# lyclyc52/Instance_NeRF

Hardware: AMD Instinct MI355X
Metric: Msamples/sec (train+infer) 3D-FRONT 800x800 at 1/2/4/8 MI355X; PSNR parity (higher is better)
Workload: dtype f32; 1 GPU; render 800x800 synthetic 3D-FRONT-like room, hash-grid NeRF L=16 F=2 T=6119864 sigma+rgb (BASELINE configs[1]), one view per step per GPU; parallelism=views sharded over 1 GPU(s), no data-path collective

## Files before the change

### include/inr.h

```cpp
#ifndef INR_H
#define INR_H

#include <stdint.h>

#ifdef __cplusplus
extern "C" {
#endif

#define INR_ABI_VERSION 13
#define INR_MAX_LEVELS 16

enum {
  INR_OK = 0,
  INR_EINVAL = -1,
  INR_ELAUNCH = -2,
  INR_ENODEV = -3
};

typedef void* inr_stream_t;

enum {
  INR_NUMERICS_TABLE_F16 = 1,
  INR_NUMERICS_MLP_F16 = 2
};

typedef struct inr_grid_desc {
  int32_t num_levels;
  int32_t level_dim;
  uint32_t offsets[INR_MAX_LEVELS + 1];
  float scales[INR_MAX_LEVELS];
  uint32_t resolutions[INR_MAX_LEVELS];
  uint32_t hashed[INR_MAX_LEVELS];
} inr_grid_desc;

int inr_abi_version(void);
const char* inr_last_error(void);
int inr_device_info(int32_t device, int64_t* props);
int inr_set_overlap_placement(int32_t on);
int inr_set_march_mode(int32_t mode);

int inr_get_rays(const float* poses, int64_t B, float fx, float fy, float cx, float cy, int32_t W,
                 const int64_t* inds , int64_t n, float* rays_o, float* rays_d, inr_stream_t s);

int inr_sample_training_batch(const float* pose , float fx, float fy, float cx, float cy, int32_t H, int32_t W,
                              const float* image , int32_t channels, const int32_t* mask ,
                              int32_t num_instances, int64_t seed, int64_t step, int64_t n, int64_t* inds ,
                              float* rays_o, float* rays_d, float* rgb , int64_t* labels ,
                              inr_stream_t s);

int inr_near_far_from_aabb(const float* rays_o, const float* rays_d, const float* aabb ,
                           int64_t N, float min_near, float* nears, float* fars, inr_stream_t s);
int inr_near_far_from_aabb_skip(const float* rays_o, const float* rays_d, const float* aabb , int64_t N,
                                float min_near, const int64_t* labels, int64_t ignore_index, float* nears, float* fars,
                                inr_stream_t s);

int inr_morton3D(const int32_t* coords , int64_t N, int32_t* indices, inr_stream_t s);
int inr_morton3D_invert(const int32_t* indices, int64_t N, int32_t* coords , inr_stream_t s);
int inr_packbits(const float* grid, int64_t n_bytes, float thresh, uint8_t* bitfield, inr_stream_t s);

int inr_mark_untrained_grid(const float* poses, int32_t B, float fx, float fy, float cx, float cy, int32_t H,
                            int32_t cascade, float bound, float* grid , inr_stream_t s);
int inr_occ_cell_positions(const int32_t* morton_idx, const float* noise, int64_t n, int32_t H, float cascade_bound,
                           float* xyz , inr_stream_t s);
int inr_occ_update(float* grid , const float* sigma , const int32_t* morton_idx ,
                   int64_t n_cells, int64_t m, float decay, float density_scale, float* tmp, double* mean_sum,
                   inr_stream_t s);
int inr_packbits_mean(const float* grid, int64_t n_cells , const double* mean_sum, float density_thresh,
                      uint8_t* bitfield, float* mean_out , const int32_t* counters ,
                      int32_t n_counters, int32_t counter_stride , double* stats_out ,
                      inr_stream_t s);
int64_t inr_occ_sample_workspace_bytes(int64_t n_cells);
int inr_occ_sample_cells(const float* grid , int64_t n_cells, const float* u ,
                         int64_t n, int32_t* morton_idx , void* workspace, inr_stream_t s);

int inr_march_write_fills_unowned_rows(int64_t N, int32_t sample_cap, int32_t max_steps);
int64_t inr_march_workspace_bytes(int64_t N, int32_t sample_cap);
int inr_march_rays_train_count(const float* rays_o, const float* rays_d, const uint8_t* bitfield,
                               float bound, float dt_gamma, int32_t max_steps, int64_t N,
                               int32_t cascade, int32_t H, const float* nears, const float* fars,
                               const float* noises , int32_t* rays ,
                               int32_t* counter , void* workspace, int32_t sample_cap, inr_stream_t s);
int inr_march_rays_train_write(const float* rays_o, const float* rays_d, const uint8_t* bitfield,
                               float bound, float dt_gamma, int32_t max_steps, int64_t N,
                               int32_t cascade, int32_t H, int64_t M, const float* nears,
                               const float* fars, const float* noises ,
                               const int32_t* rays , float* xyzs ,
                               float* dirs , float* deltas , const void* workspace,
                               int32_t sample_cap, inr_stream_t s);

int inr_march_rays_patch_write(const float* rays_o, const float* rays_d, const uint8_t* bitfield,
                               float bound, float dt_gamma, int32_t max_steps, int64_t N,
                               int32_t cascade, int32_t H, int64_t M, const float* nears,
                               const float* fars, const float* noises ,
                               const int32_t* rays ,
                               float* xyzs, float* dirs , float* deltas,
                               const void* workspace, int32_t sample_cap, int32_t* ray_ids ,
                               int32_t normalise , inr_stream_t s);
int inr_composite_rays_patch_forward(const float* sigmas, const float* rgbs, const float* deltas,
                                     const int32_t* rays, int64_t N, int64_t M, float T_thresh,
                                     const float* extra , int32_t K,
                                     float* weights_sum, float* depth, float* image,
                                     float* extra_out , float* weights ,
                                     uint64_t* skippable ,
                                     inr_stream_t s);
int inr_project_masks_patch(const float* xyzs, const float* weights, const int32_t* rays, int64_t N, int64_t M,
                            const uint32_t* mask_words, int32_t W, int32_t L, int32_t H, const float* bbox ,
                            int32_t k_total, int32_t k_base, int32_t k_count, float* out, inr_stream_t s);

int inr_march_rays(int64_t n_alive, int32_t n_step, const int32_t* rays_alive, const float* rays_t,
                   const float* rays_o, const float* rays_d, float bound, float dt_gamma,
                   int32_t max_steps, int32_t cascade, int32_t H, const uint8_t* bitfield,
                   const float* nears, const float* fars, float* xyzs, float* dirs, float* deltas,
                   inr_stream_t s);
int inr_composite_rays(int64_t n_alive, int32_t n_step, int32_t* rays_alive, float* rays_t,
                       const float* sigmas, const float* rgbs, const float* deltas,
                       float* weights_sum, float* depth, float* image, float T_thresh,
                       const float* extra , float* extra_acc ,
                       int32_t K, inr_stream_t s);
int inr_compact_alive(const int32_t* rays_alive, int64_t n_alive, int32_t* out, int32_t* n_out,
                      inr_stream_t s);

int inr_composite_rays_train_forward(const float* sigmas, const float* rgbs, const float* deltas,
                                     const int32_t* rays, int64_t N, int64_t M, float T_thresh,
                                     const float* extra , int32_t K,
                                     float* weights_sum, float* depth, float* image,
                                     float* extra_out , float* weights ,
                                     int32_t* sample_ray , inr_stream_t s);
int inr_composite_rays_extra_forward(const float* weights , const float* extra , const int32_t* rays,
                                     int64_t N, int64_t M, int32_t K, float* extra_out ,
                                     const int64_t* labels , int32_t n_classes, int64_t ignore_index,
                                     float* grad_pix, void* workspace, float* loss_out, inr_stream_t s);
int inr_composite_rays_train_backward(const float* grad_weights_sum, const float* grad_image,
                                      const float* grad_extra_out , const float* sigmas,
                                      const float* rgbs, const float* extra, const float* deltas,
                                      const int32_t* rays, const float* weights_sum,
                                      const float* image, const float* weights ,
                                      int64_t N, int64_t M, float T_thresh, int32_t K,
                                      float* grad_sigmas, float* grad_rgbs ,
                                      float* grad_extra , const int32_t* total_dev ,
                                      inr_stream_t s);

int inr_grid_encode_forward(const float* x , const float* embeddings ,
                            const inr_grid_desc* desc , int64_t M, float bound,
                            float* out , inr_stream_t s);
int inr_grid_encode_backward(const float* x, const float* grad_out ,
                             const inr_grid_desc* desc , int64_t M, float bound,
                             float* grad_embeddings , inr_stream_t s);

int inr_grid_encode_backward_ordered(const float* x, const float* grad_out, const int32_t* order,
                                     const inr_grid_desc* desc , int64_t M, float bound,
                                     float* grad_embeddings , inr_stream_t s);
int inr_grid_encode_backward_input(const float* x, const float* grad_out , const float* embeddings,
                                   const inr_grid_desc* desc , int64_t M, float bound, float* grad_x,
                                   inr_stream_t s);
int inr_grid_encode_backward_levels(const float* x, const float* grad_out, const int32_t* order,
                                    const inr_grid_desc* desc, int64_t M, float bound, float* grad_embeddings,
                                    int32_t level_lo, int32_t level_hi, inr_stream_t s);

#define INR_GRID_FX_STATE_FLOATS 4192
int inr_grid_encode_backward_levels_fx(const float* x, const float* grad_out, const int32_t* order,
                                       const inr_grid_desc* desc, int64_t M, float bound, float* grad_embeddings,
                                       int32_t level_lo, int32_t level_hi, float* fx_state ,
                                       inr_stream_t s);
int inr_grid_grad_finish_fx(float* grad_embeddings, const inr_grid_desc* desc , int32_t level_lo,
                            int32_t level_hi, float* fx_state, inr_stream_t s);
int inr_grid_fx_update(float* fx_state, int32_t num_levels, float headroom, int32_t sum_bits , inr_stream_t s);
int inr_grid_encode_backward_levels_fx64(const float* x, const float* grad_out, const int32_t* order,
                                         const inr_grid_desc* desc, int64_t M, float bound, float* grad_embeddings,
                                         int64_t* acc64 , int32_t level_lo, int32_t level_hi, float* fx_state,
                                         inr_stream_t s);
int inr_grid_grad_finish_fx64(int64_t* acc64, float* grad_embeddings, const inr_grid_desc* desc , int32_t level_lo,
                              int32_t level_hi, float* fx_state, inr_stream_t s);

int inr_sh_encode_forward(const float* d , int64_t M, int32_t degree, float* out, inr_stream_t s);
int inr_sh_encode_backward(const float* grad_out, const float* d, int64_t M, int32_t degree,
                           float* grad_d, inr_stream_t s);
int inr_sh_table_q(const float* d , int64_t N, float* out , inr_stream_t s);

int64_t inr_nerf_packed_floats(void);
int inr_nerf_pack_weights(const float* sigma_w0, const float* sigma_w1, const float* color_w0,
                          const float* color_w1, const float* color_w2, float* packed , int32_t numerics);
int64_t inr_instance_packed_floats(int32_t K);
int inr_instance_pack_weights(const float* w0, const float* w1, const float* w2, int32_t K,
                              float* packed , int32_t numerics);
int inr_nerf_forward(const float* x, const float* d, int64_t M, const int32_t* n_samples_dev,
                     float bound, const void* embeddings, const inr_grid_desc* desc ,
                     const float* packed , float density_scale, float* sigma, float* rgb,
// ... 167 lines not shown
```

### instance_nerf_amd/_lib.py

```python
import ctypes
import os
from ctypes import POINTER, Structure, c_char_p, c_float, c_int32, c_int64, c_uint32, c_void_p

import torch

_HERE = os.path.dirname(os.path.abspath(__file__))
LIB_PATH = os.environ.get("INR_LIB_PATH") or os.path.join(_HERE, "csrc", "libinr_hip.so")
MAX_LEVELS = 16
GRID_FX_STATE_FLOATS = 4192
NUMERICS_TABLE_F16, NUMERICS_MLP_F16 = 1, 2


class GridDesc(Structure):
    _fields_ = [("num_levels", c_int32), ("level_dim", c_int32),
                ("offsets", c_uint32 * (MAX_LEVELS + 1)), ("scales", c_float * MAX_LEVELS),
                ("resolutions", c_uint32 * MAX_LEVELS), ("hashed", c_uint32 * MAX_LEVELS)]


P = c_void_p
_SIGS = {
    "inr_abi_version": (c_int32, []),
    "inr_last_error": (c_char_p, []),
    "inr_set_overlap_placement": (c_int32, [c_int32]),
    "inr_set_march_mode": (c_int32, [c_int32]),
    "inr_device_info": (c_int32, [c_int32, POINTER(c_int64)]),
    "inr_get_rays": (c_int32, [P, c_int64, c_float, c_float, c_float, c_float, c_int32, P, c_int64, P, P, P]),
    "inr_sample_training_batch": (c_int32, [P, c_float, c_float, c_float, c_float, c_int32, c_int32, P, c_int32, P, c_int32,
                                            c_int64, c_int64, c_int64, P, P, P, P, P, P]),
    "inr_near_far_from_aabb": (c_int32, [P, P, P, c_int64, c_float, P, P, P]),
    "inr_near_far_from_aabb_skip": (c_int32, [P, P, P, c_int64, c_float, P, c_int64, P, P, P]),
    "inr_morton3D": (c_int32, [P, c_int64, P, P]),
    "inr_morton3D_invert": (c_int32, [P, c_int64, P, P]),
    "inr_packbits": (c_int32, [P, c_int64, c_float, P, P]),
    "inr_mark_untrained_grid": (c_int32, [P, c_int32, c_float, c_float, c_float, c_float, c_int32, c_int32, c_float, P, P]),
    "inr_occ_cell_positions": (c_int32, [P, P, c_int64, c_int32, c_float, P, P]),
    "inr_occ_update": (c_int32, [P, P, P, c_int64, c_int64, c_float, c_float, P, P, P]),
    "inr_packbits_mean": (c_int32, [P, c_int64, P, c_float, P, P, P, c_int32, c_int32, P, P]),
    "inr_occ_sample_workspace_bytes": (c_int64, [c_int64]),
    "inr_occ_sample_cells": (c_int32, [P, c_int64, P, c_int64, P, P, P]),
    "inr_march_write_fills_unowned_rows": (c_int32, [c_int64, c_int32, c_int32]),
    "inr_march_workspace_bytes": (c_int64, [c_int64, c_int32]),
    "inr_march_rays_train_count": (c_int32, [P, P, P, c_float, c_float, c_int32, c_int64, c_int32, c_int32,
                                             P, P, P, P, P, P, c_int32, P]),
    "inr_march_rays_train_write": (c_int32, [P, P, P, c_float, c_float, c_int32, c_int64, c_int32, c_int32,
                                             c_int64, P, P, P, P, P, P, P, P, c_int32, P]),
    "inr_march_rays_patch_write": (c_int32, [P, P, P, c_float, c_float, c_int32, c_int64, c_int32, c_int32,
                                             c_int64, P, P, P, P, P, P, P, P, c_int32, P, c_int32, P]),
    "inr_nerf_bwd_packed_floats": (c_int64, []),
    "inr_nerf_pack_weights_device": (c_int32, [P, P, P, P, P, P, P, P]),
    "inr_nerf_forward_train": (c_int32, [P, P, c_int64, c_float, P, POINTER(GridDesc), P, P, P, P, P, P, P, P, P, P]),
    "inr_nerf_backward": (c_int32, [P, P, P, P, P, P, P, c_int64, c_float, P, P, P, P, P, P, P, P]),
    "inr_instance_bwd_packed_floats": (c_int64, []),
    "inr_instance_pack_weights_device": (c_int32, [P, P, P, c_int32, P, P, P]),
    "inr_instance_forward_train": (c_int32, [P, c_int64, c_float, P, POINTER(GridDesc), P, c_int32, P, P, P, P, P]),
    "inr_instance_backward": (c_int32, [P, c_int32, P, P, c_int64, P, P, P, P, P]),
    "inr_nerf_forward_enc": (c_int32, [P, P, c_int64, c_float, P, POINTER(GridDesc), P, P, P, P, P]),
    "inr_nerf_head_backward": (c_int32, [P, P, P, P, c_int64, c_float, P, P, P, P, P, P, P, P, P, P, c_int64, P]),
    "inr_instance_forward_enc": (c_int32, [P, c_int64, P, c_float, P, POINTER(GridDesc), P, c_int32, P, P, P]),
    "inr_instance_head_workspace_bytes": (c_int64, []),
    "inr_instance_head_backward": (c_int32, [P, P, P, P, c_int32, c_int64, c_int64, P, P, P, P, P, P, P, P, P, P, P, c_int64, P]),
    "inr_adam_step_multi": (c_int32, [c_int32, P, P, P, P, P, P, c_float, c_float, c_float, c_int32, c_float, P]),
    "inr_adam_ema_step_multi": (c_int32, [c_int32, P, P, P, P, P, P, c_float, c_float, c_float, c_int32, c_float, P,
                                          c_float, P]),
    "inr_adam_set_hyper": (c_int32, [P, c_int32, c_float, c_float, c_float, c_int32, P, P]),
    "inr_adam_step_multi_dev": (c_int32, [c_int32, P, P, P, P, P, P, c_float, c_float, c_float, P]),
    "inr_copy_multi": (c_int32, [c_int32, P, P, P, P]),
    "inr_adam_set_hyper_ema": (c_int32, [P, c_int32, c_float, c_float, c_float, c_int32, c_float, P, P]),
    "inr_adam_ema_step_multi_dev": (c_int32, [c_int32, P, P, P, P, P, P, c_float, c_float, c_float, P, P]),
    "inr_cross_entropy": (c_int32, [P, P, c_int64, c_int32, c_int64, P, P, P, P]),
    "inr_finish_rays": (c_int32, [P, P, P, P, P, P, c_float, c_float, c_float, c_int64, P, P, P]),
    "inr_finish_rays_mse": (c_int32, [P, P, P, P, P, c_float, c_float, c_float, P, P, c_int64, P, P, P, P, P]),
    "inr_sh_table_q": (c_int32, [P, c_int64, P, P]),
    "inr_nerf_forward_table": (c_int32, [P, P, P, c_int64, c_float, P, POINTER(GridDesc), P, c_float, P, P, c_int32, P]),
    "inr_nerf_forward_table_sliced_workspace_bytes": (c_int64, [c_int64]),
    "inr_nerf_forward_table_sliced": (c_int32, [P, P, P, c_int64, c_float, P, POINTER(GridDesc), P, c_float, P, P, P, P]),
    "inr_composite_rays_patch_forward": (c_int32, [P, P, P, P, c_int64, c_int64, c_float, P, c_int32, P, P, P, P, P, P, P]),
    "inr_project_masks_patch": (c_int32, [P, P, P, c_int64, c_int64, P, c_int32, c_int32, c_int32, P, c_int32, c_int32, c_int32,
                                          P, P]),
    "inr_march_rays": (c_int32, [c_int64, c_int32, P, P, P, P, c_float, c_float, c_int32, c_int32, c_int32,
                                 P, P, P, P, P, P, P]),
    "inr_composite_rays": (c_int32, [c_int64, c_int32, P, P, P, P, P, P, P, P, c_float, P, P, c_int32, P]),
    "inr_compact_alive": (c_int32, [P, c_int64, P, P, P]),
    "inr_composite_rays_extra_forward": (c_int32, [P, P, P, c_int64, c_int64, c_int32, P, P, c_int32, c_int64, P, P, P, P]),
    "inr_composite_rays_train_forward": (c_int32, [P, P, P, P, c_int64, c_int64, c_float, P, c_int32, P, P, P, P, P, P, P]),
    "inr_composite_rays_train_backward": (c_int32, [P, P, P, P, P, P, P, P, P, P, P, c_int64, c_int64, c_float, c_int32,
                                                    P, P, P, P, P]),
    "inr_grid_encode_forward": (c_int32, [P, P, POINTER(GridDesc), c_int64, c_float, P, P]),
    "inr_grid_encode_backward": (c_int32, [P, P, POINTER(GridDesc), c_int64, c_float, P, P]),
    "inr_grid_encode_backward_ordered": (c_int32, [P, P, P, POINTER(GridDesc), c_int64, c_float, P, P]),
    "inr_grid_encode_backward_input": (c_int32, [P, P, P, POINTER(GridDesc), c_int64, c_float, P, P]),
    "inr_grid_encode_backward_levels": (c_int32, [P, P, P, POINTER(GridDesc), c_int64, c_float, P, c_int32, c_int32, P]),
    "inr_grid_encode_backward_levels_fx": (c_int32, [P, P, P, POINTER(GridDesc), c_int64, c_float, P, c_int32, c_int32, P, P]),
    "inr_grid_grad_finish_fx": (c_int32, [P, POINTER(GridDesc), c_int32, c_int32, P, P]),
    "inr_grid_fx_update": (c_int32, [P, c_int32, c_float, c_int32, P]),
    "inr_grid_encode_backward_levels_fx64": (c_int32, [P, P, P, POINTER(GridDesc), c_int64, c_float, P, P, c_int32, c_int32, P, P]),
    "inr_grid_grad_finish_fx64": (c_int32, [P, P, POINTER(GridDesc), c_int32, c_int32, P, P]),
    "inr_sh_encode_forward": (c_int32, [P, c_int64, c_int32, P, P]),
    "inr_sh_encode_backward": (c_int32, [P, P, c_int64, c_int32, P, P]),
    "inr_nerf_packed_floats": (c_int64, []),
    "inr_nerf_pack_weights": (c_int32, [P, P, P, P, P, P, c_int32]),
    "inr_instance_packed_floats": (c_int64, [c_int32]),
    "inr_instance_pack_weights": (c_int32, [P, P, P, c_int32, P, c_int32]),
    "inr_nerf_forward": (c_int32, [P, P, c_int64, P, c_float, P, POINTER(GridDesc), P, c_float, P, P, P, c_int32, P]),
    "inr_nerf_forward_dirs": (c_int32, [P, c_int64, c_float, P, POINTER(GridDesc), P, P, c_int32, P, P]),
    "inr_nerf_forward_lattice": (c_int32, [P, P, P, c_int32, c_int32, c_int32, c_float, P, POINTER(GridDesc), P, P, c_int32,
                                           c_float, P, P]),
    "inr_instance_forward": (c_int32, [P, c_int64, P, c_float, P, POINTER(GridDesc), P, c_int32, P, P]),
    "inr_instance_lattice": (c_int32, [P, P, P, c_int32, c_int32, c_int32, c_float, P, POINTER(GridDesc), P, c_float,
                                       c_float, P, POINTER(GridDesc), P, c_int32, P, P, P, P]),
    "inr_instance_volume_stats": (c_int32, [P, P, c_int32, c_int32, c_int32, c_int32, P, c_int64, P, P, P, P]),
    "inr_mesh_workspace_bytes": (c_int64, [c_int32, c_int32, c_int32, c_int32]),
    "inr_mesh_count": (c_int32, [P, c_int32, c_float, c_float, P, c_int32, c_int32, c_int32, c_int32, c_int32, P, c_int64, P, P]),
    "inr_mesh_emit": (c_int32, [P, c_int32, c_float, c_float, P, c_int32, P, P, P, P, c_int32, c_int32, c_int32, c_float,
                                c_float, c_float, c_int32, P, c_int64, c_int32, c_int32, P, P, P, P, P]),
    "inr_components_workspace_bytes": (c_int64, [c_int32, c_int32, c_int32]),
    "inr_components_label": (c_int32, [P, c_int32, c_int32, c_int32, c_int32, P, c_int64, P, P]),
    "inr_components_filter": (c_int32, [P, P, P, c_int32, c_int32, c_int32, c_int32, c_int32, c_int32, c_int32, P, c_int64,
                                        P, P, P, P, P, P]),
    "inr_pack_mask_bits": (c_int32, [P, P, c_int64, c_int32, c_float, c_int64, P, P]),
    "inr_match_count": (c_int32, [P, P, c_int64, c_int64, c_int32, c_int32, P, P, P, P, P]),
    "inr_match_assign": (c_int32, [P, P, P, P, P, c_int64, c_int64, c_int32, c_int32, P, P, P, P]),
    "inr_roi_align_3d_set_mode": (c_int32, [c_int32]),
    "inr_roi_align_3d_forward": (c_int32, [P, P, P, c_int32, c_int32, c_int32, c_int32, c_int32, c_int64, c_int32,
                                           c_int32, c_int32, c_float, P, P]),
    "inr_roi_align_3d_backward": (c_int32, [P, P, P, c_int32, c_int32, c_int32, c_int32, c_int32, c_int64, c_int32,
                                            c_int32, c_int32, c_float, P, P]),
    "inr_roi_align_3d_backward_workspace_bytes": (c_int64, [c_int32, c_int32, c_int32, c_int32, c_int32, c_int64, c_int32,
                                                            c_int32, c_int32]),
    "inr_roi_align_3d_backward_prefers_workspace": (c_int32, [c_int32, c_int32, c_int32, c_int32, c_int32, c_int64, c_int32,
                                                              c_int32, c_int32, c_int64]),
    "inr_roi_align_3d_backward_ws": (c_int32, [P, P, P, c_int32, c_int32, c_int32, c_int32, c_int32, c_int64, c_int32,
                                               c_int32, c_int32, c_float, P, P, c_int64, P]),
    "inr_nerf_render": (c_int32, [P, P, P, P, c_int64, c_int64, c_float, P, POINTER(GridDesc), P, c_float, c_float,
                                  P, P, P, P, P, c_int32, c_int32, P]),
    "inr_instance_render": (c_int32, [P, P, P, c_int64, c_int64, c_float, P, POINTER(GridDesc), P, c_int32, P, c_int32, P,
                                      c_int32, P]),
    "inr_linear_wgrad_workspace_bytes": (c_int64, []),
    "inr_linear_wgrad": (c_int32, [P, P, c_int64, c_int32, c_int32, P, P, P]),
    "inr_adam_step": (c_int32, [P, P, P, P, c_int64, c_float, c_float, c_float, c_float, c_int32, c_float, P]),
}
EXPORTS = tuple(_SIGS)

ABI_VERSION = 13
INSTANCE_STATS_WORKSPACE_BYTES = 512 * 64 * 8 * 4
_lib = None


def load():
    global _lib
    if _lib is not None:
        return _lib
    if not os.path.exists(LIB_PATH):
        raise RuntimeError(
            f"{LIB_PATH} is missing: build it with `python -m instance_nerf_amd.build` "
            "(or __graft_entry__.build()).  There is no CPU fallback.")
    lib = ctypes.CDLL(LIB_PATH)
    version = getattr(lib, "inr_abi_version", None)
    if version is not None:
        version.restype, version.argtypes = c_int32, []
# ... 61 lines not shown
```

### instance_nerf_amd/csrc/raymarch.hip

```cpp
#include "common.h"

namespace inr {

static thread_local char g_err[512] = "";
int g_field_lds_min = 0;
int g_march_lds_pad = 0;
void set_error(const char* fmt, ...) {
  va_list ap;
  va_start(ap, fmt);
  vsnprintf(g_err, sizeof(g_err), fmt, ap);
  va_end(ap);
}

constexpr int kRayBlock = 256;
constexpr float kSqrt3x2 = 3.4641016151377544f;

__global__ void __launch_bounds__(kRayBlock) k_near_far(const float* __restrict__ rays_o,
                                                        const float* __restrict__ rays_d,
                                                        const float* __restrict__ aabb, int64_t N,
                                                        float min_near, float* __restrict__ nears,
                                                        float* __restrict__ fars,
                                                        const int64_t* __restrict__ labels, int64_t ignore) {
  const int64_t n = (int64_t)blockIdx.x * blockDim.x + threadIdx.x;
  if (n >= N) return;
  float near = -INFINITY, far = INFINITY;
  bool miss = labels != nullptr && labels[n] == ignore;
#pragma unroll
  for (int a = 0; a < 3; ++a) {
    const float o = rays_o[n * 3 + a];
    const float rd = 1.0f / rays_d[n * 3 + a];
    const float t0 = (aabb[a] - o) * rd;
    const float t1 = (aabb[a + 3] - o) * rd;
    const float lo = t0 > t1 ? t1 : t0;
    const float hi = t0 > t1 ? t0 : t1;
    if (a > 0) miss = miss || (near > hi) || (lo > far);
    near = lo > near ? lo : near;
    far = hi < far ? hi : far;
  }
  if (near < min_near) near = min_near;
  nears[n] = miss ? 3.402823466e+38f : near;
  fars[n] = miss ? 3.402823466e+38f : far;
}

__global__ void __launch_bounds__(kRayBlock) k_get_rays(const float* __restrict__ poses, int64_t B, float fx, float fy,
                                                        float cx, float cy, int W, const int64_t* __restrict__ inds,
                                                        int64_t n, float* __restrict__ rays_o,
                                                        float* __restrict__ rays_d) {
  const int64_t idx = (int64_t)blockIdx.x * blockDim.x + threadIdx.x;
  if (idx >= B * n) return;
  const int64_t b = idx / n, k = idx - b * n;
  const int64_t pix = inds ? inds[k] : k;
  const float i = (float)(pix % W) + 0.5f, j = (float)(pix / W) + 0.5f;
  const float xs = (i - cx) / fx, ys = (j - cy) / fy;
  const float nrm = sqrtf(xs * xs + ys * ys + 1.0f * 1.0f);
  const float dx = xs / nrm, dy = ys / nrm, dz = 1.0f / nrm;
  const float* P = poses + b * 16;
#pragma unroll
  for (int r = 0; r < 3; ++r) {
    rays_d[idx * 3 + r] = dx * P[r * 4 + 0] + dy * P[r * 4 + 1] + dz * P[r * 4 + 2];
    rays_o[idx * 3 + r] = P[r * 4 + 3];
  }
}

__device__ __forceinline__ uint64_t mix64(uint64_t z) {
  z = (z ^ (z >> 30)) * 0xBF58476D1CE4E5B9ull;
  z = (z ^ (z >> 27)) * 0x94D049BB133111EBull;
  return z ^ (z >> 31);
}
__global__ void __launch_bounds__(kRayBlock) k_sample_batch(const float* __restrict__ pose, float fx, float fy, float cx,
                                                            float cy, int H, int W, const float* __restrict__ image,
                                                            int C, const int32_t* __restrict__ mask, int num_instances,
                                                            uint64_t seed, uint64_t step, int64_t n,
                                                            int64_t* __restrict__ inds, float* __restrict__ rays_o,
                                                            float* __restrict__ rays_d, float* __restrict__ rgb,
                                                            int64_t* __restrict__ labels) {
  const int64_t k = (int64_t)blockIdx.x * blockDim.x + threadIdx.x;
  if (k >= n) return;
  const uint64_t h = mix64(seed + 0x9E3779B97F4A7C15ull * ((step << 32) + (uint64_t)k));
  const uint64_t pix = ((h >> 32) * (uint64_t)((int64_t)H * W)) >> 32;
  inds[k] = (int64_t)pix;
  const float i = (float)(pix % (uint64_t)W) + 0.5f, j = (float)(pix / (uint64_t)W) + 0.5f;
  const float xs = (i - cx) / fx, ys = (j - cy) / fy;
  const float nrm = sqrtf(xs * xs + ys * ys + 1.0f * 1.0f);
  const float dx = xs / nrm, dy = ys / nrm, dz = 1.0f / nrm;
#pragma unroll
  for (int r = 0; r < 3; ++r) {
    rays_d[k * 3 + r] = dx * pose[r * 4 + 0] + dy * pose[r * 4 + 1] + dz * pose[r * 4 + 2];
    rays_o[k * 3 + r] = pose[r * 4 + 3];
  }
  if (image) {
    for (int c = 0; c < C; ++c) rgb[k * C + c] = image[pix * C + c];
  }
  if (mask) {
    const int32_t l = mask[pix];
    labels[k] = l >= num_instances ? -1 : (int64_t)l;
  }
}

__global__ void k_morton3D(const int32_t* __restrict__ coords, int64_t N, int32_t* __restrict__ out) {
  const int64_t n = (int64_t)blockIdx.x * blockDim.x + threadIdx.x;
  if (n >= N) return;
  out[n] = (int32_t)morton3((uint32_t)coords[n * 3], (uint32_t)coords[n * 3 + 1], (uint32_t)coords[n * 3 + 2]);
}
__global__ void k_morton3D_invert(const int32_t* __restrict__ idx, int64_t N, int32_t* __restrict__ coords) {
  const int64_t n = (int64_t)blockIdx.x * blockDim.x + threadIdx.x;
  if (n >= N) return;
  const uint32_t m = (uint32_t)idx[n];
  coords[n * 3 + 0] = (int32_t)compact_bits10(m);
  coords[n * 3 + 1] = (int32_t)compact_bits10(m >> 1);
  coords[n * 3 + 2] = (int32_t)compact_bits10(m >> 2);
}
__global__ void k_packbits(const float* __restrict__ grid, int64_t n_bytes, float thresh,
                           uint8_t* __restrict__ bits) {
  const int64_t n = (int64_t)blockIdx.x * blockDim.x + threadIdx.x;
  if (n >= n_bytes) return;
  const float4 a = reinterpret_cast<const float4*>(grid)[n * 2];
  const float4 b = reinterpret_cast<const float4*>(grid)[n * 2 + 1];
  uint32_t v = (a.x > thresh) | ((a.y > thresh) << 1) | ((a.z > thresh) << 2) | ((a.w > thresh) << 3) |
               ((b.x > thresh) << 4) | ((b.y > thresh) << 5) | ((b.z > thresh) << 6) | ((b.w > thresh) << 7);
  bits[n] = (uint8_t)v;
}

__global__ void k_occ_positions(const int32_t* __restrict__ morton, const float* __restrict__ noise, int64_t n, float Hm1,
                                float ext, float half, float* __restrict__ xyz) {
// ... 119 lines not shown
  }
};

struct MortonCalc {
  __device__ __forceinline__ uint32_t operator()(uint32_t x, uint32_t y, uint32_t z) const { return morton3(x, y, z); }
};
struct MortonLut {
  const uint32_t* lut;
  __device__ __forceinline__ uint32_t operator()(uint32_t x, uint32_t y, uint32_t z) const {
    return lut[x] | (lut[y] << 1) | (lut[z] << 2);
  }
};

template <bool kSingle = false, bool kConstDt = false, class Emit, class Advance, class Morton = MortonCalc>
__device__ __forceinline__ int march_ray(const MarchParams& P, const Ray& r, float t, float far,
                                         int max_emit, Emit&& emit, Advance&& advance, Morton morton = Morton()) {
  int n = 0;
  float last_t = t;
  const StepRule<kConstDt> step(P);
  const float mb1 = fminf(ldexpf(1.0f, 0), P.bound), rmb1 = 1.0f / mb1;
  while (t < far && n < max_emit) {
    const float px = clampf(r.ox + t * r.dx, -P.bound, P.bound);
    const float py = clampf(r.oy + t * r.dy, -P.bound, P.bound);
    const float pz = clampf(r.oz + t * r.dz, -P.bound, P.bound);
    const float dt = step(P, t);
    int level = 0;
    float mb = mb1, rmb = rmb1;
    if constexpr (!kSingle) {
      int e0, e1;
      (void)frexpf(fmaxf(fabsf(px), fmaxf(fabsf(py), fabsf(pz))), &e0);
      (void)frexpf(dt * (float)P.H * 0.5f, &e1);
      level = max(clampi(e0, 0, P.C - 1), clampi(e1, 0, P.C - 1));
      mb = fminf(ldexpf(1.0f, level), P.bound);
      rmb = 1.0f / mb;
    }
    const int nx = clampi((int)(((px * rmb + 1.0f) * 0.5f) * (float)P.H), 0, P.H - 1);
    const int ny = clampi((int)(((py * rmb + 1.0f) * 0.5f) * (float)P.H), 0, P.H - 1);
    const int nz = clampi((int)(((pz * rmb + 1.0f) * 0.5f) * (float)P.H), 0, P.H - 1);
    const uint32_t idx = (uint32_t)level * (uint32_t)P.H3 + morton((uint32_t)nx, (uint32_t)ny, (uint32_t)nz);
    const bool occ = (P.bits[idx >> 3] >> (idx & 7)) & 1;
    if (occ) {
      const float tn = t + dt;
      emit(px, py, pz, dt, tn - last_t, t);
      t = tn;
      advance();
      last_t = tn;
      ++n;
    } else {
      const float ax = ((float)nx + 0.5f) + 0.5f * r.sx;
      const float ay = ((float)ny + 0.5f) + 0.5f * r.sy;
      const float az = ((float)nz + 0.5f) + 0.5f * r.sz;
      const float cx = (((ax * P.rH) * 2.0f - 1.0f) * mb - px) * r.rdx;
      const float cy = (((ay * P.rH) * 2.0f - 1.0f) * mb - py) * r.rdy;
      const float cz = (((az * P.rH) * 2.0f - 1.0f) * mb - pz) * r.rdz;
      const float tt = t + fmaxf(0.0f, fminf(cx, fminf(cy, cz)));
      do {
        t = t + step(P, t);
        advance();
      } while (t < tt);
    }
  }
  return n;
}
template <class Emit>
__device__ __forceinline__ int march_ray(const MarchParams& P, const Ray& r, float t, float far,
                                         int max_emit, Emit&& emit) {
  return P.dt_gamma == 0.0f ? march_ray<false, true>(P, r, t, far, max_emit, emit, [] {})
                            : march_ray<false, false>(P, r, t, far, max_emit, emit, [] {});
}
template <class Emit, class Advance, class Morton>
__device__ __forceinline__ int march_ray_any(const MarchParams& P, const Ray& r, float t, float far,
                                             int max_emit, Emit&& emit, Advance&& advance, Morton morton) {
  if (P.dt_gamma == 0.0f)
    return P.C == 1 ? march_ray<true, true>(P, r, t, far, max_emit, emit, advance, morton)
                    : march_ray<false, true>(P, r, t, far, max_emit, emit, advance, morton);
  return P.C == 1 ? march_ray<true, false>(P, r, t, far, max_emit, emit, advance, morton)
                  : march_ray<false, false>(P, r, t, far, max_emit, emit, advance, morton);
}

__device__ __forceinline__ float start_t(const MarchParams& P, float near, float noise) {
  return near + step_dt(P, near) * noise;
}

__global__ void __launch_bounds__(kRayBlock) k_march_count(MarchParams P, const float* __restrict__ rays_o,
                                                           const float* __restrict__ rays_d, int64_t N,
                                                           int max_steps, const float* __restrict__ nears,
                                                           const float* __restrict__ fars,
                                                           const float* __restrict__ noises,
                                                           int32_t* __restrict__ counts,
                                                           int32_t* __restrict__ block_sums,
                                                           uint32_t* __restrict__ mask, int cap_words) {
  __shared__ int32_t wsum[kRayBlock / 64];
  __shared__ uint32_t lut[1024];
  for (int i = threadIdx.x; i < P.H; i += kRayBlock) lut[i] = expand_bits10((uint32_t)i);
  __syncthreads();
  const MortonLut morton{lut};
  const int64_t n = (int64_t)blockIdx.x * blockDim.x + threadIdx.x;
  int cnt = 0;
  if (n < N) {
    const Ray r = load_ray(rays_o, rays_d, n);
    const float t0 = start_t(P, nears[n], noises ? noises[n] : 0.0f);
    if (cap_words > 0) {
      uint32_t word = 0;
      int widx = 0, cand = 0;
      bool ok = true;
      cnt = march_ray_any(P, r, t0, fars[n], max_steps,
                      [&](float, float, float, float, float, float) {
                        const int w = cand >> 5;
                        if (w < cap_words) {
                          while (widx < w) {
                            mask[(int64_t)widx * N + n] = word;
                            word = 0;
                            ++widx;
                          }
                          word |= 1u << (cand & 31);
                        } else {
                          ok = false;
                        }
                      },
                      [&] { ++cand; }, morton);
      if (widx < cap_words) mask[(int64_t)widx * N + n] = word;
      mask[(int64_t)cap_words * N + n] = ok ? 1u : 0u;
    } else {
      cnt = march_ray_any(P, r, t0, fars[n], max_steps, [](float, float, float, float, float, float) {}, [] {}, morton);
    }
    counts[n] = cnt;
  }
  const int incl = wave_inclusive_scan(cnt);
  if ((threadIdx.x & 63) == 63) wsum[threadIdx.x >> 6] = incl;
  __syncthreads();
  if (threadIdx.x == 0) {
    int s = 0;
#pragma unroll
    for (int w = 0; w < kRayBlock / 64; ++w) s += wsum[w];
    block_sums[blockIdx.x] = s;
  }
}

__global__ void __launch_bounds__(1024) k_scan_block_sums(int32_t* __restrict__ block_sums, int n_blocks,
                                                          int64_t N, int32_t* __restrict__ counter) {
  __shared__ int32_t wsum[16];
  __shared__ int32_t carry_s;
  if (threadIdx.x == 0) carry_s = 0;
  __syncthreads();
  for (int base = 0; base < n_blocks; base += 1024) {
    const int i = base + threadIdx.x;
    const int v = i < n_blocks ? block_sums[i] : 0;
    const int incl = wave_inclusive_scan(v);
    if ((threadIdx.x & 63) == 63) wsum[threadIdx.x >> 6] = incl;
    __syncthreads();
    int wave_off = 0;
    for (int w = 0; w < (int)(threadIdx.x >> 6); ++w) wave_off += wsum[w];
    const int carry = carry_s;
    if (i < n_blocks) block_sums[i] = carry + wave_off + incl - v;
    __syncthreads();
    if (threadIdx.x == 1023) carry_s = carry + wave_off + incl;
    __syncthreads();
  }
  if (threadIdx.x == 0) {
    counter[0] = carry_s;
    counter[1] = (int32_t)N;
  }
}

__global__ void __launch_bounds__(kRayBlock) k_finalize_offsets(const int32_t* __restrict__ counts,
                                                                const int32_t* __restrict__ block_prefix,
                                                                int64_t N, int32_t* __restrict__ rays) {
  __shared__ int32_t wsum[kRayBlock / 64];
  const int64_t n = (int64_t)blockIdx.x * blockDim.x + threadIdx.x;
  const int cnt = n < N ? counts[n] : 0;
  const int incl = wave_inclusive_scan(cnt);
  if ((threadIdx.x & 63) == 63) wsum[threadIdx.x >> 6] = incl;
  __syncthreads();
  int off = block_prefix[blockIdx.x] + incl - cnt;
  for (int w = 0; w < (int)(threadIdx.x >> 6); ++w) off += wsum[w];
  if (n < N) {
    rays[n * 3 + 0] = (int32_t)n;
    rays[n * 3 + 1] = off;
    rays[n * 3 + 2] = cnt;
  }
}

template <bool kConstDt, class Emit>
__device__ __forceinline__ void replay_ray_t(const MarchParams& P, const Ray& r, const uint32_t* __restrict__ mask, int64_t N,
                                             int64_t n, float t, int cnt, Emit&& emit) {
  const StepRule<kConstDt> step(P);
  float last_t = t;
  int emitted = 0;
  for (int w = 0; emitted < cnt; ++w) {
    const uint32_t bits = mask[(int64_t)w * N + n];
    for (int b0 = 0; b0 < 32; b0 += 8) {
      const uint32_t sub = (bits >> b0) & 0xFFu;
      if (__ballot(sub != 0u) == 0ull) {
#pragma unroll
        for (int j = 0; j < 8; ++j) t = t + step(P, t);
        continue;
      }
#pragma unroll
      for (int j = 0; j < 8; ++j) {
        const float dt = step(P, t);
        const float tn = t + dt;
        if (sub & (1u << j)) {
          const float px = clampf(r.ox + t * r.dx, -P.bound, P.bound);
          const float py = clampf(r.oy + t * r.dy, -P.bound, P.bound);
          const float pz = clampf(r.oz + t * r.dz, -P.bound, P.bound);
          emit(px, py, pz, dt, tn - last_t, t);
          last_t = tn;
// ... 358 lines not shown
  }
  if (threadIdx.x == 0) {
    counter[0] = carry_s;
    counter[1] = (int32_t)N;
  }
}

__global__ void __launch_bounds__(kCoopRaysPerBlock * 64) k_march_write_coop(MarchParams P, const float* __restrict__ rays_o,
                                                                             const float* __restrict__ rays_d, int64_t N,
                                                                             int64_t M, const float* __restrict__ nears,
                                                                             const float* __restrict__ fars,
                                                                             const float* __restrict__ noises,
                                                                             const int32_t* __restrict__ rays,
                                                                             float* __restrict__ xyzs, float* __restrict__ dirs,
                                                                             float* __restrict__ deltas) {
  const int64_t n = (int64_t)blockIdx.x * kCoopRaysPerBlock + (threadIdx.x >> 6);
  if (n >= N) return;
  const int off = rays[n * 3 + 1];
  const int cnt = rays[n * 3 + 2];
  if (cnt == 0 || (int64_t)off + cnt > M) return;
  const Ray r = load_ray(rays_o, rays_d, n);
  const float t0 = start_t(P, nears[n], noises ? noises[n] : 0.0f);
  auto put = [&](int k, float px, float py, float pz, float dt, float delta, float) {
    const int64_t i = (int64_t)off + k;
    xyzs[i * 3 + 0] = px; xyzs[i * 3 + 1] = py; xyzs[i * 3 + 2] = pz;
    dirs[i * 3 + 0] = r.dx; dirs[i * 3 + 1] = r.dy; dirs[i * 3 + 2] = r.dz;
    deltas[i * 2 + 0] = dt; deltas[i * 2 + 1] = delta;
  };
  if (P.C == 1) march_ray_coop<true>(P, r, t0, fars[n], cnt, put);
  else march_ray_coop<false>(P, r, t0, fars[n], cnt, put);
}

constexpr int kCeBlocks = 64;
__global__ void __launch_bounds__(256) k_ce_rows(const float* __restrict__ logits, const int64_t* __restrict__ labels,
                                                 int64_t N, int K, int64_t ignore_index, float* __restrict__ dlogits,
                                                 float2* __restrict__ part) {
  __shared__ float2 red[4];
  const int lane = threadIdx.x & 63;
  const int64_t wave = ((int64_t)blockIdx.x * blockDim.x + threadIdx.x) >> 6;
  const int64_t n_waves = ((int64_t)gridDim.x * blockDim.x) >> 6;
  float loss_sum = 0.f, kept = 0.f, bad = 0.f;
  for (int64_t r = wave; r < N; r += n_waves) {
    const int64_t y = labels[r];
    const bool keep = y != ignore_index && y >= 0 && y < K;
    if (y != ignore_index && !(y >= 0 && y < K)) bad += 1.f;
    const float x = lane < K ? logits[r * K + lane] : -INFINITY;
    float m = x;
#pragma unroll
    for (int d = 1; d < 64; d <<= 1) m = fmaxf(m, __shfl_xor(m, d, 64));
    const float e = lane < K ? expf(x - m) : 0.f;
    float ssum = e;
#pragma unroll
    for (int d = 1; d < 64; d <<= 1) ssum += __shfl_xor(ssum, d, 64);
    const float xy = __shfl(x, keep ? (int)y : 0, 64);
    if (keep) {
      loss_sum += (m + logf(ssum)) - xy;
      kept += 1.f;
    }
    if (lane < K) dlogits[r * K + lane] = keep ? e / ssum - (lane == (int)y ? 1.f : 0.f) : 0.f;
  }
  if (bad > 0.f) loss_sum = NAN;
  if (lane == 0) red[threadIdx.x >> 6] = make_float2(loss_sum, kept);
  __syncthreads();
  if (threadIdx.x == 0)
    part[blockIdx.x] = make_float2(red[0].x + red[1].x + red[2].x + red[3].x, red[0].y + red[1].y + red[2].y + red[3].y);
}
__global__ void __launch_bounds__(256) k_ce_scale(float* __restrict__ dlogits, int64_t n, const float2* __restrict__ part,
                                                  int n_part, float* __restrict__ loss) {
  float sum = 0.f, kept = 0.f;
  for (int i = 0; i < n_part; ++i) {
    const float2 p = part[i];
    sum += p.x;
    kept += p.y;
  }
  const float inv = kept > 0.f ? 1.0f / kept : 0.f;
  for (int64_t i = (int64_t)blockIdx.x * blockDim.x + threadIdx.x; i < n; i += (int64_t)gridDim.x * blockDim.x) dlogits[i] *= inv;
  if (blockIdx.x == 0 && threadIdx.x == 0) *loss = sum / kept;
}

__global__ void __launch_bounds__(256) k_finish_rays(const float* image, const float* depth,
                                                     const float* __restrict__ weights_sum,
                                                     const float* __restrict__ nears, const float* __restrict__ fars,
                                                     const float* __restrict__ t0, float bg_r, float bg_g, float bg_b,
                                                     int64_t N, float* image_out, float* depth_out) {
  const int64_t n = (int64_t)blockIdx.x * blockDim.x + threadIdx.x;
  if (n >= N) return;
  const float ws = weights_sum[n];
  const float a = 1.0f - ws;
  image_out[n * 3 + 0] = image[n * 3 + 0] + a * bg_r;
  image_out[n * 3 + 1] = image[n * 3 + 1] + a * bg_g;
  image_out[n * 3 + 2] = image[n * 3 + 2] + a * bg_b;
  float d = depth[n];
  if (t0) d = d + t0[n] * ws;
  depth_out[n] = fmaxf(d - nears[n], 0.0f) / (fars[n] - nears[n]);
}

constexpr int kFinishMseThreads = 1024;
__global__ void __launch_bounds__(kFinishMseThreads) k_finish_rays_mse(
    const float* __restrict__ image, const float* __restrict__ depth, const float* __restrict__ weights_sum,
    const float* __restrict__ nears, const float* __restrict__ fars, float bg_r, float bg_g, float bg_b,
    const float* __restrict__ bg_rays, const float* __restrict__ target, int64_t N, float* __restrict__ image_out,
    float* __restrict__ depth_out, float* __restrict__ grad, float* __restrict__ loss) {
  __shared__ float part[kFinishMseThreads / 64];
  const float inv = 1.0f / (3.0f * (float)N);
  float acc = 0.0f;
  for (int64_t n = threadIdx.x; n < N; n += kFinishMseThreads) {
    const float ws = weights_sum[n];
    const float a = 1.0f - ws;
    float bg[3] = {bg_r, bg_g, bg_b};
    if (bg_rays) { bg[0] = bg_rays[n * 3 + 0]; bg[1] = bg_rays[n * 3 + 1]; bg[2] = bg_rays[n * 3 + 2]; }
    float gws = 0.0f;
#pragma unroll
    for (int c = 0; c < 3; ++c) {
      const float px = image[n * 3 + c] + a * bg[c];
      const float e = px - target[n * 3 + c];
      const float g = 2.0f * e * inv;
      image_out[n * 3 + c] = px;
      grad[n * 3 + c] = g;
      gws -= g * bg[c];
      acc += e * e;
    }
    grad[3 * N + n] = gws;
    depth_out[n] = fmaxf(depth[n] - nears[n], 0.0f) / (fars[n] - nears[n]);
  }
  for (int o = 32; o > 0; o >>= 1) acc += __shfl_xor(acc, o, 64);
  if ((threadIdx.x & 63) == 0) part[threadIdx.x >> 6] = acc;
  __syncthreads();
  if (threadIdx.x == 0) {
    float t = 0.0f;
    for (int w = 0; w < kFinishMseThreads / 64; ++w) t += part[w];
    loss[0] = t * inv;
  }
}

__global__ void __launch_bounds__(kRayBlock) k_march_rays(MarchParams P, int64_t n_alive, int n_step,
                                                          const int32_t* __restrict__ rays_alive,
                                                          const float* __restrict__ rays_t,
                                                          const float* __restrict__ rays_o,
                                                          const float* __restrict__ rays_d,
                                                          const float* __restrict__ fars,
                                                          float* __restrict__ xyzs, float* __restrict__ dirs,
                                                          float* __restrict__ deltas) {
  const int64_t n = (int64_t)blockIdx.x * blockDim.x + threadIdx.x;
  if (n >= n_alive) return;
  const int64_t base = n * n_step;
  const int32_t ridx = rays_alive[n];
  int written = 0;
  if (ridx >= 0) {
    const Ray r = load_ray(rays_o, rays_d, ridx);
    int64_t i = base;
    written = march_ray(P, r, rays_t[ridx], fars[ridx], n_step,
                        [&](float px, float py, float pz, float dt, float delta, float) {
                          xyzs[i * 3 + 0] = px; xyzs[i * 3 + 1] = py; xyzs[i * 3 + 2] = pz;
                          dirs[i * 3 + 0] = r.dx; dirs[i * 3 + 1] = r.dy; dirs[i * 3 + 2] = r.dz;
                          deltas[i * 2 + 0] = dt; deltas[i * 2 + 1] = delta;
                          ++i;
                        });
  }
  for (int64_t i = base + written; i < base + n_step; ++i) {
    xyzs[i * 3 + 0] = 0.f; xyzs[i * 3 + 1] = 0.f; xyzs[i * 3 + 2] = 0.f;
    dirs[i * 3 + 0] = 0.f; dirs[i * 3 + 1] = 0.f; dirs[i * 3 + 2] = 0.f;
    deltas[i * 2 + 0] = 0.f; deltas[i * 2 + 1] = 0.f;
  }
}

__global__ void __launch_bounds__(kRayBlock) k_composite_rays(int64_t n_alive, int n_step,
                                                              int32_t* __restrict__ rays_alive,
                                                              float* __restrict__ rays_t,
                                                              const float* __restrict__ sigmas,
                                                              const float* __restrict__ rgbs,
                                                              const float* __restrict__ deltas,
                                                              float* __restrict__ weights_sum,
                                                              float* __restrict__ depth, float* __restrict__ image,
                                                              float T_thresh, const float* __restrict__ extra,
                                                              float* __restrict__ extra_acc, int K) {
  const int64_t n = (int64_t)blockIdx.x * blockDim.x + threadIdx.x;
  if (n >= n_alive) return;
// ... 274 lines not shown
    if (lane == 0) Pprev = 1.0f;
    const float T = T_carry * Pprev, Tn = T_carry * P;
    const bool used = act && (T >= T_thresh || (base + lane) == 0);
    const float w = used ? alpha * T : 0.0f;
    const float ar = cr_carry + wave_incl_sum(w * cr, lane);
    const float ag = cg_carry + wave_incl_sum(w * cg, lane);
    const float ab = cb_carry + wave_incl_sum(w * cb, lane);
    if (act) {
      grad_rgbs[i * 3] = gr * w; grad_rgbs[i * 3 + 1] = gg * w; grad_rgbs[i * 3 + 2] = gb * w;
      grad_sigmas[i] = used ? d0 * (gr * (Tn * cr - (rf - ar)) + gg * (Tn * cg - (gf - ag)) + gb * (Tn * cb - (bf - ab)) +
                                    gw * (1.0f - wsf))
                            : 0.0f;
    }
    T_carry *= __shfl(P, 63, 64);
    cr_carry = __shfl(ar, 63, 64); cg_carry = __shfl(ag, 63, 64); cb_carry = __shfl(ab, 63, 64);
    if (T_carry < T_thresh) dead = true;
  }
}

__global__ void __launch_bounds__(kRayBlock) k_composite_train_extra_bwd(
    const float* __restrict__ g_extra_out, const float* __restrict__ wbuf, const int32_t* __restrict__ rays, int64_t N,
    int64_t M, int K, float* __restrict__ grad_extra) {
  const int64_t n = ((int64_t)blockIdx.x * blockDim.x + threadIdx.x) >> 6;
  const int lane = threadIdx.x & 63;
  if (n >= N) return;
  const int32_t rid = rays[n * 3], off = rays[n * 3 + 1];
  int32_t cnt = rays[n * 3 + 2];
  if ((int64_t)off + cnt > M) cnt = 0;
  if (lane >= K) return;
  const float g = g_extra_out[(int64_t)rid * K + lane];
  for (int s = 0; s < cnt; ++s) grad_extra[((int64_t)off + s) * K + lane] = wbuf[(int64_t)off + s] * g;
}

constexpr int kGroup = 16;

struct GroupCursor {
  int c[kGroup];
  int S;
  int r;
  int k;
  __device__ __forceinline__ void init(int my_count, int my_offset) {
    const int lane = threadIdx.x & 63, g0 = lane & ~(kGroup - 1);
    r = lane & (kGroup - 1);
#pragma unroll
    for (int i = 0; i < kGroup; ++i) c[i] = __shfl(my_count, g0 + i, 64);
    S = __shfl(my_offset, g0, 64);
    k = 0;
  }
  __device__ __forceinline__ int total() const {
    int t = 0;
#pragma unroll
    for (int i = 0; i < kGroup; ++i) t += c[i];
    return t;
  }
  int nact_ = 0, rank_ = 0, k_change_ = 0;
  __device__ __forceinline__ int next() {
    if (k >= k_change_) {
      int nact = 0, rank = 0, nxt = 0x7FFFFFFF;
#pragma unroll
      for (int i = 0; i < kGroup; ++i) {
        const bool gt = c[i] > k;
        nact += gt ? 1 : 0;
        rank += (gt && i < r) ? 1 : 0;
        nxt = gt ? min(nxt, c[i]) : nxt;
      }
      nact_ = nact; rank_ = rank; k_change_ = nxt;
    }
    const int slot = S + rank_;
    S += nact_;
    ++k;
    return slot;
  }
};

__global__ void __launch_bounds__(kRayBlock) k_march_write_patch(MarchParams P, const float* __restrict__ rays_o,
                                                                 const float* __restrict__ rays_d, int64_t N, int64_t M,
                                                                 const float* __restrict__ nears,
                                                                 const float* __restrict__ fars,
                                                                 const float* __restrict__ noises,
                                                                 const int32_t* __restrict__ rays,
                                                                 float* __restrict__ xyzs, float* __restrict__ dirs,
                                                                 float* __restrict__ deltas,
                                                                 const uint32_t* __restrict__ mask, int cap_words,
                                                                 int32_t* __restrict__ ray_ids, int normalise) {
  const int64_t n = (int64_t)blockIdx.x * blockDim.x + threadIdx.x;
  const int off = n < N ? rays[n * 3 + 1] : 0;
  const int cnt = n < N ? rays[n * 3 + 2] : 0;
  GroupCursor cur;
  cur.init(cnt, off);
  if (cnt == 0 || (int64_t)cur.S + cur.total() > M) return;
  const Ray r = load_ray(rays_o, rays_d, n);
  const float rb = 2.0f * P.bound;
  auto emit = [&](float px, float py, float pz, float dt, float delta, float) {
    const int64_t i = cur.next();
    if (normalise) {
      px = (px + P.bound) / rb; py = (py + P.bound) / rb; pz = (pz + P.bound) / rb;
    }
    xyzs[i * 3 + 0] = px; xyzs[i * 3 + 1] = py; xyzs[i * 3 + 2] = pz;
    if (dirs) { dirs[i * 3 + 0] = r.dx; dirs[i * 3 + 1] = r.dy; dirs[i * 3 + 2] = r.dz; }
    if (ray_ids) ray_ids[i] = (int32_t)n;
    deltas[i * 2 + 0] = dt; deltas[i * 2 + 1] = delta;
  };
  const float t0 = start_t(P, nears[n], noises ? noises[n] : 0.0f);
  if (cap_words > 0 && mask[(int64_t)cap_words * N + n]) {
    replay_ray(P, r, mask, N, n, t0, cnt, emit);
  } else {
    march_ray(P, r, t0, fars[n], cnt, emit);
  }
}

__global__ void __launch_bounds__(kRayBlock) k_composite_patch_fwd(const float* __restrict__ sigmas,
                                                                   const float* __restrict__ rgbs,
                                                                   const float* __restrict__ deltas,
                                                                   const int32_t* __restrict__ rays, int64_t N, int64_t M,
                                                                   float T_thresh, float* __restrict__ wbuf,
                                                                   float* __restrict__ weights_sum,
                                                                   float* __restrict__ depth, float* __restrict__ image,
                                                                   unsigned long long* __restrict__ skippable) {
  const int64_t n = (int64_t)blockIdx.x * blockDim.x + threadIdx.x;
  const int lane = threadIdx.x & 63, g0 = lane & ~(kGroup - 1), rr = lane & (kGroup - 1);
  const int32_t rid = n < N ? rays[n * 3] : 0;
  const int off = n < N ? rays[n * 3 + 1] : 0;
  int cnt = n < N ? rays[n * 3 + 2] : 0;
  int S = __shfl(off, g0, 64);
  int gtot = cnt;
#pragma unroll
  for (int d = 1; d < kGroup; d <<= 1) gtot += __shfl_xor(gtot, d, 64);
  if ((int64_t)S + gtot > M) cnt = 0;
  int maxc = cnt;
#pragma unroll
  for (int d = 1; d < 64; d <<= 1) maxc = max(maxc, __shfl_xor(maxc, d, 64));
  float T = 1.0f, r = 0, g = 0, b = 0, ws = 0, t = 0, dsum = 0;
  bool done = false;
  unsigned n_skip = 0;
  constexpr int kAhead = 8;
  for (int k = 0; k < maxc; k += kAhead) {
    unsigned field[kAhead];
    int64_t slot[kAhead];
    bool active[kAhead];
    float2 dl[kAhead];
    float sg[kAhead], cr[kAhead], cg[kAhead], cb[kAhead];
#pragma unroll
    for (int j = 0; j < kAhead; ++j) {
      active[j] = k + j < cnt;
      field[j] = (unsigned)(__ballot(active[j]) >> g0) & 0xFFFFu;
      slot[j] = (int64_t)S + __popc(field[j] & ((1u << rr) - 1u));
      S += __popc(field[j]);
      const int64_t i = (active[j] && !done) ? slot[j] : 0;
      dl[j] = reinterpret_cast<const float2*>(deltas)[i];
      sg[j] = sigmas[i];
      cr[j] = rgbs[i * 3]; cg[j] = rgbs[i * 3 + 1]; cb[j] = rgbs[i * 3 + 2];
    }
#pragma unroll
    for (int j = 0; j < kAhead; ++j) {
      if (skippable) {
        const unsigned live = (unsigned)(__ballot(active[j] && !done) >> g0) & 0xFFFFu;
        if (rr == 0 && field[j] != 0 && live == 0) n_skip += __popc(field[j]);
      }
      if (active[j] && !done) {
        const float alpha = 1.0f - expf(-sg[j] * dl[j].x);
        const float w = alpha * T;
        r += w * cr[j]; g += w * cg[j]; b += w * cb[j];
        t += dl[j].y;
        dsum += w * t;
        ws += w;
        if (wbuf) wbuf[slot[j]] = w;
        T *= 1.0f - alpha;
        if (T < T_thresh) done = true;
      } else if (active[j] && wbuf) {
        wbuf[slot[j]] = 0.0f;
      }
    }
  }
  if (n < N) {
    weights_sum[rid] = ws; depth[rid] = dsum;
    image[rid * 3] = r; image[rid * 3 + 1] = g; image[rid * 3 + 2] = b;
  }
  if (skippable) {
#pragma unroll
    for (int d = 1; d < 64; d <<= 1) n_skip += __shfl_xor(n_skip, d, 64);
    if (lane == 0 && n_skip) atomicAdd(skippable, (unsigned long long)n_skip);
  }
}

__global__ void __launch_bounds__(kRayBlock) k_composite_patch_extra(const float* __restrict__ wbuf,
                                                                     const float* __restrict__ extra,
                                                                     const int32_t* __restrict__ rays, int64_t N,
                                                                     int64_t M, int K, float* __restrict__ extra_out) {
  const int64_t n = ((int64_t)blockIdx.x * blockDim.x + threadIdx.x) >> 6;
  const int lane = threadIdx.x & 63;
  if (n >= N) return;
  const int64_t g0 = n & ~(int64_t)(kGroup - 1);
  const int r = (int)(n - g0);
  int c[kGroup];
  int total = 0;
#pragma unroll
  for (int i = 0; i < kGroup; ++i) {
    c[i] = (g0 + i < N) ? rays[(g0 + i) * 3 + 2] : 0;
    total += c[i];
  }
  const int32_t rid = rays[n * 3];
  int64_t S = rays[g0 * 3 + 1];
  const int cnt = (S + total <= M) ? c[r] : 0;
  float acc = 0.0f;
  for (int k = 0; k < cnt; ++k) {
    int nact = 0, rank = 0;
#pragma unroll
    for (int i = 0; i < kGroup; ++i) {
      const int gt = c[i] > k ? 1 : 0;
      nact += gt;
      rank += (i < r) ? gt : 0;
    }
    const int64_t slot = S + rank;
    S += nact;
    const float w = wbuf[slot];
    if (lane < K && w != 0.0f) acc += w * extra[slot * K + lane];
  }
  if (lane < K) extra_out[(int64_t)rid * K + lane] = acc;
}

struct MaskVolume {
  float lo[3], hi[3], res[3];
  int W, L, H;
};
__global__ void __launch_bounds__(kRayBlock) k_project_masks_patch(const float* __restrict__ xyzs,
                                                                   const float* __restrict__ wbuf,
                                                                   const int32_t* __restrict__ rays, int64_t N, int64_t M,
                                                                   const uint32_t* __restrict__ words, MaskVolume V,
                                                                   int k_total, int k_base, int k_count,
                                                                   float* __restrict__ out) {
  const int64_t n = (int64_t)blockIdx.x * blockDim.x + threadIdx.x;
  const int lane = threadIdx.x & 63, g0 = lane & ~(kGroup - 1), rr = lane & (kGroup - 1);
  const int32_t rid = n < N ? rays[n * 3] : 0;
  const int off = n < N ? rays[n * 3 + 1] : 0;
  int cnt = n < N ? rays[n * 3 + 2] : 0;
  int S = __shfl(off, g0, 64);
  int gtot = cnt;
#pragma unroll
  for (int d = 1; d < kGroup; d <<= 1) gtot += __shfl_xor(gtot, d, 64);
  if ((int64_t)S + gtot > M) cnt = 0;
  int maxc = cnt;
#pragma unroll
  for (int d = 1; d < 64; d <<= 1) maxc = max(maxc, __shfl_xor(maxc, d, 64));
  float acc[32];
#pragma unroll
  for (int i = 0; i < 32; ++i) acc[i] = 0.0f;
  for (int k = 0; k < maxc; ++k) {
    const bool active = k < cnt;
    const unsigned field = (unsigned)(__ballot(active) >> g0) & 0xFFFFu;
    const int64_t slot = (int64_t)S + __popc(field & ((1u << rr) - 1u));
    S += __popc(field);
    const float w = active ? wbuf[slot] : 0.0f;
    if (w != 0.0f) {
      const float x = xyzs[slot * 3], y = xyzs[slot * 3 + 1], z = xyzs[slot * 3 + 2];
      const float fx = floorf(((x - V.lo[0]) / (V.hi[0] - V.lo[0])) * V.res[0]);
      const float fy = floorf(((y - V.lo[1]) / (V.hi[1] - V.lo[1])) * V.res[1]);
      const float fz = floorf(((z - V.lo[2]) / (V.hi[2] - V.lo[2])) * V.res[2]);
      const bool inside = fx >= 0.0f && fx < V.res[0] && fy >= 0.0f && fy < V.res[1] && fz >= 0.0f && fz < V.res[2];
      if (inside) {
        const uint32_t word = words[((int64_t)(int)fx * V.L + (int)fy) * V.H + (int)fz];
#pragma unroll
        for (int i = 0; i < 32; ++i) acc[i] += ((word >> i) & 1u) ? w : 0.0f;
      }
    }
  }
  if (n < N) {
    float* dst = out + (int64_t)rid * k_total + k_base;
#pragma unroll
    for (int i = 0; i < 32; ++i)
      if (i < k_count) dst[i] = acc[i];
  }
}

static MarchParams make_params(const uint8_t* bits, float bound, float dt_gamma, int max_steps, int C, int H) {
  MarchParams P;
  P.bits = bits;
  P.bound = bound;
  P.dt_gamma = dt_gamma;
  P.dt_min = kSqrt3x2 / (float)max_steps;
  P.dt_max = kSqrt3x2 * (float)(1 << (C - 1)) / (float)H;
  P.rH = (float)(1.0 / H);
  P.C = C;
  P.H = H;
  P.H3 = H * H * H;
  return P;
}

}

using namespace inr;

extern "C" {

int inr_abi_version(void) { return INR_ABI_VERSION; }
const char* inr_last_error(void) { return inr::g_err; }

int inr_set_overlap_placement(int32_t on) {
  INR_REQUIRE(on >= 0, "on must be 0 (off), 1 (on) or an LDS byte count >= 1024");
  INR_REQUIRE(on <= 1 || on >= 1024, "on must be 0 (off), 1 (on) or an LDS byte count >= 1024");
  inr::g_field_lds_min = on >= 1024 ? on : on ? 84 * 1024 : 0;
  inr::g_march_lds_pad = on ? 48 * 1024 : 0;
// ... 129 lines not shown

int inr_packbits_mean(const float* grid, int64_t n_cells, const double* mean_sum, float density_thresh, uint8_t* bitfield,
                      float* mean_out, const int32_t* counters, int32_t n_counters, int32_t counter_stride,
                      double* stats_out, inr_stream_t s) {
  INR_REQUIRE(n_cells > 0 && n_cells % 8 == 0 && grid && mean_sum && bitfield, "bad argument");
  INR_REQUIRE(((uintptr_t)grid & 15) == 0, "grid must be 16-byte aligned");
  INR_REQUIRE(n_counters >= 0 && (n_counters == 0 || (counters && stats_out && counter_stride > 0)), "bad counters");
  k_packbits_mean<<<blocks_for(n_cells / 8, 256), 256, 0, as_stream(s)>>>(grid, n_cells / 8, mean_sum, 1.0 / (double)n_cells,
                                                                           density_thresh, bitfield, mean_out, counters,
                                                                           n_counters, counter_stride, stats_out);
  return check_launch("packbits_mean");
}

int64_t inr_occ_sample_workspace_bytes(int64_t n_cells) {
  if (n_cells <= 0) return -1;
  const int64_t n_blocks = (n_cells + kOccBlockCells - 1) / kOccBlockCells;
  return n_blocks * (kOccBlockCells / 64) * (int64_t)sizeof(uint64_t) + (n_blocks + 2 * kOccBuckets) * (int64_t)sizeof(int32_t);
}

int inr_occ_sample_cells(const float* grid, int64_t n_cells, const float* u, int64_t n, int32_t* morton_idx,
                         void* workspace, inr_stream_t s) {
  INR_REQUIRE(grid && u && morton_idx && workspace && n > 0 && n_cells > 0, "bad argument");
  INR_REQUIRE(2 * n < (int64_t)1 << 31 && n_cells < (int64_t)1 << 31, "sizes must fit int32");
  INR_REQUIRE(((uintptr_t)workspace & 7) == 0, "workspace must be 8-byte aligned");
  const int64_t n_blocks = (n_cells + kOccBlockCells - 1) / kOccBlockCells;
  INR_REQUIRE(n_blocks <= kOccMaxBlocks, "grid too large for the block table (H <= 256)");
  hipStream_t st = as_stream(s);
  uint64_t* masks = reinterpret_cast<uint64_t*>(workspace);
  int32_t* block_counts = reinterpret_cast<int32_t*>(masks + n_blocks * (kOccBlockCells / 64));
  int32_t* hist = block_counts + n_blocks;
  k_occ_count<<<(int)n_blocks, kOccBlockCells, 0, st>>>(grid, n_cells, masks, block_counts, hist);
  k_occ_hist<<<(int)std::min<int64_t>(64, blocks_for(2 * n, 1024)), 1024, 0, st>>>(u, n, hist);
  const size_t lds = (size_t)(2 * (kOccBuckets + 1) + n_blocks + 1) * sizeof(int32_t);
  static size_t lds_allowed = 64 * 1024;
  if (lds > lds_allowed) {
    if (hipFuncSetAttribute((const void*)k_occ_pick, hipFuncAttributeMaxDynamicSharedMemorySize, (int)lds) != hipSuccess) {
      set_error("occ_sample_cells: %zu bytes of LDS refused", lds);
      return INR_ELAUNCH;
    }
    lds_allowed = lds;
  }
  k_occ_pick<<<(int)std::min<int64_t>(256, blocks_for(2 * n, 1024)), 1024, lds, st>>>(u + 2 * n, n, hist, masks, block_counts,
                                                                                       (int)n_blocks, n_cells, morton_idx);
  return check_launch("occ_sample_cells");
}

static int g_march_mode = -1;
static bool use_coop(int64_t N, int32_t sample_cap) {
  if (sample_cap > 0) return false;
  if (g_march_mode >= 0) return g_march_mode != 0;
  return N <= 32768;
}
int inr_set_march_mode(int32_t mode) {
  INR_REQUIRE(mode >= -1 && mode <= 1, "mode must be -1 (automatic), 0 (lane per ray) or 1 (wave per ray)");
  g_march_mode = mode;
  return INR_OK;
}

static int64_t ws_ints(int64_t N) {
  const int64_t nb = (N + kRayBlock - 1) / kRayBlock;
  return ((N + nb + 64 + 1) / 2) * 2;
}
static int cap_words_of(int32_t sample_cap) { return sample_cap > 0 ? (sample_cap + 31) / 32 : 0; }
constexpr int kStagePitch = 1024;
constexpr int64_t kStageMaxRays = 8192;
static bool use_stage(int64_t N, int32_t sample_cap, int max_steps) {
  return use_coop(N, sample_cap) && N <= kStageMaxRays && max_steps <= kStagePitch;
}
static int64_t stage_offset_bytes(int64_t N, int32_t sample_cap) {
  const int w = cap_words_of(sample_cap);
  const int64_t b = ws_ints(N) * (int64_t)sizeof(int32_t) + (w ? N * (int64_t)(w + 1) * (int64_t)sizeof(uint32_t) : 0);
  return (b + 15) / 16 * 16;
}
int inr_march_write_fills_unowned_rows(int64_t N, int32_t sample_cap, int32_t max_steps) {
  return use_stage(N, sample_cap, max_steps) ? 1 : 0;
}
int64_t inr_march_workspace_bytes(int64_t N, int32_t sample_cap) {
  const int64_t base = stage_offset_bytes(N, sample_cap);
  return base + (N <= kStageMaxRays && sample_cap == 0 ? N * (int64_t)kStagePitch * 5 * (int64_t)sizeof(float) : 0);
}

static size_t march_lds_pad() { return (size_t)inr::g_march_lds_pad; }

int inr_march_rays_train_count(const float* rays_o, const float* rays_d, const uint8_t* bitfield, float bound,
                               float dt_gamma, int32_t max_steps, int64_t N, int32_t cascade, int32_t H,
                               const float* nears, const float* fars, const float* noises, int32_t* rays,
                               int32_t* counter, void* workspace, int32_t sample_cap, inr_stream_t s) {
  INR_REQUIRE(rays_o && rays_d && bitfield && nears && fars && rays && counter && workspace, "null pointer");
  INR_REQUIRE(N > 0 && N < (1ll << 31), "N out of range");
  INR_REQUIRE(max_steps > 0 && cascade >= 1 && H >= 8 && H <= 1024, "bad grid parameters");
  const MarchParams P = make_params(bitfield, bound, dt_gamma, max_steps, cascade, H);
  const unsigned nb = blocks_for(N, kRayBlock);
  INR_REQUIRE(sample_cap >= 0 && ((uintptr_t)workspace & 7) == 0, "workspace must be 8-byte aligned");
  int32_t* counts = reinterpret_cast<int32_t*>(workspace);
  int32_t* block_sums = counts + N;
  uint32_t* mask = reinterpret_cast<uint32_t*>(counts + ws_ints(N));
  hipStream_t st = as_stream(s);
  if (use_coop(N, sample_cap)) {
    float* stage = use_stage(N, sample_cap, max_steps)
                       ? reinterpret_cast<float*>(reinterpret_cast<char*>(workspace) + stage_offset_bytes(N, sample_cap)) : nullptr;
    k_march_count_coop<<<blocks_for(N, kCoopRaysPerBlock), kCoopRaysPerBlock * 64, 0, st>>>(P, rays_o, rays_d, N, max_steps,
                                                                                          nears, fars, noises, counts, stage,
                                                                                          kStagePitch);
    k_scan_counts<<<1, 1024, 0, st>>>(counts, N, rays, counter);
    return check_launch("march_rays_train_count");
  }
  k_march_count<<<nb, kRayBlock, march_lds_pad(), st>>>(P, rays_o, rays_d, N, max_steps, nears, fars, noises, counts, block_sums,
                                          mask, cap_words_of(sample_cap));
  k_scan_block_sums<<<1, 1024, 0, st>>>(block_sums, (int)nb, N, counter);
  k_finalize_offsets<<<nb, kRayBlock, 0, st>>>(counts, block_sums, N, rays);
  return check_launch("march_rays_train_count");
}

int inr_march_rays_train_write(const float* rays_o, const float* rays_d, const uint8_t* bitfield, float bound,
                               float dt_gamma, int32_t max_steps, int64_t N, int32_t cascade, int32_t H, int64_t M,
                               const float* nears, const float* fars, const float* noises, const int32_t* rays,
                               float* xyzs, float* dirs, float* deltas, const void* workspace, int32_t sample_cap,
                               inr_stream_t s) {
  INR_REQUIRE(rays_o && rays_d && bitfield && nears && fars && rays, "null pointer");
  INR_REQUIRE(N > 0 && M >= 0, "bad sizes");
  if (M == 0) return INR_OK;
  INR_REQUIRE(M == 0 || (xyzs && dirs && deltas), "null output");
  const MarchParams P = make_params(bitfield, bound, dt_gamma, max_steps, cascade, H);
  INR_REQUIRE(sample_cap == 0 || workspace, "sample_cap > 0 needs the workspace of the count pass");
  const uint32_t* mask = sample_cap > 0 ? reinterpret_cast<const uint32_t*>(reinterpret_cast<const int32_t*>(workspace) + ws_ints(N)) : nullptr;
  if (use_stage(N, sample_cap, max_steps)) {
    INR_REQUIRE(workspace, "the staged marcher needs the workspace of the count pass");
    const float* stage = reinterpret_cast<const float*>(reinterpret_cast<const char*>(workspace) + stage_offset_bytes(N, sample_cap));
    k_march_write_staged<<<blocks_for(N, kCoopRaysPerBlock), kCoopRaysPerBlock * 64, 0, as_stream(s)>>>(
        rays_d, N, M, rays, stage, kStagePitch, xyzs, dirs, deltas);
    return check_launch("march_rays_train_write");
  }
  if (use_coop(N, sample_cap)) {
    k_march_write_coop<<<blocks_for(N, kCoopRaysPerBlock), kCoopRaysPerBlock * 64, 0, as_stream(s)>>>(
        P, rays_o, rays_d, N, M, nears, fars, noises, rays, xyzs, dirs, deltas);
    return check_launch("march_rays_train_write");
  }
  k_march_write<<<blocks_for(N, kRayBlock), kRayBlock, 0, as_stream(s)>>>(P, rays_o, rays_d, N, M, nears, fars, noises,
                                                                          rays, xyzs, dirs, deltas, mask, cap_words_of(sample_cap));
  return check_launch("march_rays_train_write");
}

int inr_march_rays_patch_write(const float* rays_o, const float* rays_d, const uint8_t* bitfield, float bound,
                               float dt_gamma, int32_t max_steps, int64_t N, int32_t cascade, int32_t H, int64_t M,
                               const float* nears, const float* fars, const float* noises, const int32_t* rays,
                               float* xyzs, float* dirs, float* deltas, const void* workspace, int32_t sample_cap,
                               int32_t* ray_ids, int32_t normalise, inr_stream_t s) {
  INR_REQUIRE(rays_o && rays_d && bitfield && nears && fars && rays, "null pointer");
  INR_REQUIRE(N > 0 && M >= 0, "bad sizes");
  if (M == 0) return INR_OK;
  INR_REQUIRE(M == 0 || (xyzs && deltas && (dirs || ray_ids)), "null output");
  const MarchParams P = make_params(bitfield, bound, dt_gamma, max_steps, cascade, H);
  INR_REQUIRE(sample_cap == 0 || workspace, "sample_cap > 0 needs the workspace of the count pass");
  const uint32_t* mask = sample_cap > 0 ? reinterpret_cast<const uint32_t*>(reinterpret_cast<const int32_t*>(workspace) + ws_ints(N)) : nullptr;
  k_march_write_patch<<<blocks_for(N, kRayBlock), kRayBlock, march_lds_pad(), as_stream(s)>>>(P, rays_o, rays_d, N, M, nears, fars,
                                                                                noises, rays, xyzs, dirs, deltas, mask,
                                                                                cap_words_of(sample_cap), ray_ids, normalise);
  return check_launch("march_rays_patch_write");
}

int inr_composite_rays_patch_forward(const float* sigmas, const float* rgbs, const float* deltas, const int32_t* rays,
                                     int64_t N, int64_t M, float T_thresh, const float* extra, int32_t K,
                                     float* weights_sum, float* depth, float* image, float* extra_out,
                                     float* weights, uint64_t* skippable, inr_stream_t s) {
  INR_REQUIRE(N >= 0 && M >= 0, "bad sizes");
  if (N == 0) return INR_OK;
  INR_REQUIRE(rays && weights_sum && depth && image, "null pointer");
  INR_REQUIRE(M == 0 || (sigmas && rgbs && deltas), "null sample arrays");
  INR_REQUIRE(!extra || (extra_out && weights && K > 0 && K <= 64), "extra needs extra_out, weights and 0 < K <= 64");
  INR_REQUIRE(((uintptr_t)deltas & 7) == 0, "deltas must be 8-byte aligned");
  hipStream_t st = as_stream(s);
  k_composite_patch_fwd<<<blocks_for(N, kRayBlock), kRayBlock, 0, st>>>(sigmas, rgbs, deltas, rays, N, M, T_thresh,
                                                                        weights, weights_sum, depth, image,
                                                                        reinterpret_cast<unsigned long long*>(skippable));
  if (extra_out && K > 0)
    k_composite_patch_extra<<<blocks_for(N * 64, kRayBlock), kRayBlock, 0, st>>>(weights, extra, rays, N, M, K,
                                                                                 extra_out);
  return check_launch("composite_rays_patch_forward");
}

int inr_project_masks_patch(const float* xyzs, const float* weights, const int32_t* rays, int64_t N, int64_t M,
                            const uint32_t* mask_words, int32_t W, int32_t L, int32_t H, const float* bbox ,
                            int32_t k_total, int32_t k_base, int32_t k_count, float* out, inr_stream_t s) {
  INR_REQUIRE(N >= 0 && M >= 0 && W > 0 && L > 0 && H > 0, "bad sizes");
  INR_REQUIRE(k_total > 0 && k_base >= 0 && k_count > 0 && k_count <= 32 && k_base + k_count <= k_total, "bad mask range");
  if (N == 0) return INR_OK;
  INR_REQUIRE(rays && mask_words && bbox && out, "null pointer");
  INR_REQUIRE(M == 0 || (xyzs && weights), "null sample arrays");
  MaskVolume V;
  for (int a = 0; a < 3; ++a) { V.lo[a] = bbox[a]; V.hi[a] = bbox[3 + a]; }
  V.res[0] = (float)W; V.res[1] = (float)L; V.res[2] = (float)H;
  V.W = W; V.L = L; V.H = H;
  k_project_masks_patch<<<blocks_for(N, kRayBlock), kRayBlock, 0, as_stream(s)>>>(xyzs, weights, rays, N, M, mask_words, V,
                                                                                 k_total, k_base, k_count, out);
  return check_launch("project_masks_patch");
}

int inr_march_rays(int64_t n_alive, int32_t n_step, const int32_t* rays_alive, const float* rays_t,
                   const float* rays_o, const float* rays_d, float bound, float dt_gamma, int32_t max_steps,
                   int32_t cascade, int32_t H, const uint8_t* bitfield, const float* nears, const float* fars,
                   float* xyzs, float* dirs, float* deltas, inr_stream_t s) {
  (void)nears;
  INR_REQUIRE(rays_alive && rays_t && rays_o && rays_d && bitfield && fars && xyzs && dirs && deltas, "null pointer");
  INR_REQUIRE(n_alive >= 0 && n_step > 0, "bad sizes");
  if (n_alive == 0) return INR_OK;
  const MarchParams P = make_params(bitfield, bound, dt_gamma, max_steps, cascade, H);
  k_march_rays<<<blocks_for(n_alive, kRayBlock), kRayBlock, 0, as_stream(s)>>>(P, n_alive, n_step, rays_alive, rays_t,
                                                                               rays_o, rays_d, fars, xyzs, dirs, deltas);
  return check_launch("march_rays");
}

int inr_composite_rays(int64_t n_alive, int32_t n_step, int32_t* rays_alive, float* rays_t, const float* sigmas,
                       const float* rgbs, const float* deltas, float* weights_sum, float* depth, float* image,
                       float T_thresh, const float* extra, float* extra_acc, int32_t K, inr_stream_t s) {
  INR_REQUIRE(rays_alive && rays_t && sigmas && rgbs && deltas && weights_sum && depth && image, "null pointer");
  INR_REQUIRE(!extra || (extra_acc && K > 0), "extra given without extra_acc/K");
  if (n_alive == 0) return INR_OK;
  k_composite_rays<<<blocks_for(n_alive, kRayBlock), kRayBlock, 0, as_stream(s)>>>(
      n_alive, n_step, rays_alive, rays_t, sigmas, rgbs, deltas, weights_sum, depth, image, T_thresh, extra, extra_acc, K);
  return check_launch("composite_rays");
}

int inr_compact_alive(const int32_t* rays_alive, int64_t n_alive, int32_t* out, int32_t* n_out, inr_stream_t s) {
  INR_REQUIRE(rays_alive && out && n_out && n_alive >= 0, "bad argument");
  if (n_alive == 0) {
    (void)hipMemsetAsync(n_out, 0, 2 * sizeof(int32_t), as_stream(s));
    return check_launch("compact_alive");
  }
  const unsigned nb = blocks_for(n_alive, kRayBlock);
  int32_t* counts = out + n_alive;
  int32_t* block_sums = counts + n_alive;
  hipStream_t st = as_stream(s);
  k_alive_flags<<<nb, kRayBlock, 0, st>>>(rays_alive, n_alive, counts, block_sums);
  k_scan_block_sums<<<1, 1024, 0, st>>>(block_sums, (int)nb, n_alive, n_out);
  k_alive_scatter<<<nb, kRayBlock, 0, st>>>(rays_alive, n_alive, block_sums, out);
  return check_launch("compact_alive");
}

int inr_cross_entropy(const float* logits, const int64_t* labels, int64_t N, int32_t K, int64_t ignore_index,
                      float* grad_logits, float* acc, float* loss, inr_stream_t s) {
  INR_REQUIRE(N >= 0 && K > 0 && K <= 64, "K must be in 1..64");
  INR_REQUIRE(acc && loss && ((uintptr_t)acc & 7) == 0, "null or misaligned pointer");
  hipStream_t st = as_stream(s);
  int nb = 0;
  if (N > 0) {
    INR_REQUIRE(logits && labels && grad_logits, "null pointer");
    nb = (int)std::min<int64_t>((N + 3) / 4, kCeBlocks);
    k_ce_rows<<<nb, 256, 0, st>>>(logits, labels, N, K, ignore_index, grad_logits, reinterpret_cast<float2*>(acc));
  }
  const unsigned nb2 = (unsigned)std::max<int64_t>(1, std::min<int64_t>((N * K + 255) / 256, (int64_t)cu_count() * 4));
  k_ce_scale<<<nb2, 256, 0, st>>>(grad_logits, N * K, reinterpret_cast<const float2*>(acc), nb, loss);
  return check_launch("cross_entropy");
}

int inr_finish_rays(const float* image, const float* depth, const float* weights_sum, const float* nears,
                    const float* fars, const float* t0, float bg_r, float bg_g, float bg_b, int64_t N, float* image_out,
                    float* depth_out, inr_stream_t s) {
  INR_REQUIRE(N >= 0, "negative N");
  if (N == 0) return INR_OK;
  INR_REQUIRE(image && depth && weights_sum && nears && fars && image_out && depth_out, "null pointer");
  k_finish_rays<<<blocks_for(N, 256), 256, 0, as_stream(s)>>>(image, depth, weights_sum, nears, fars, t0, bg_r, bg_g, bg_b,
                                                              N, image_out, depth_out);
  return check_launch("finish_rays");
}

int inr_finish_rays_mse(const float* image, const float* depth, const float* weights_sum, const float* nears,
                        const float* fars, float bg_r, float bg_g, float bg_b, const float* bg_rays, const float* target,
                        int64_t N, float* image_out, float* depth_out, float* grad, float* loss, inr_stream_t s) {
  INR_REQUIRE(N > 0 && N <= INR_FINISH_MSE_MAX_RAYS, "N out of range (one workgroup: 0 < N <= INR_FINISH_MSE_MAX_RAYS)");
  INR_REQUIRE(image && depth && weights_sum && nears && fars && target && image_out && depth_out && grad && loss,
              "null pointer");
  k_finish_rays_mse<<<1, kFinishMseThreads, 0, as_stream(s)>>>(image, depth, weights_sum, nears, fars, bg_r, bg_g, bg_b,
                                                               bg_rays, target, N, image_out, depth_out, grad, loss);
  return check_launch("finish_rays_mse");
}

int inr_composite_rays_train_forward(const float* sigmas, const float* rgbs, const float* deltas, const int32_t* rays,
                                     int64_t N, int64_t M, float T_thresh, const float* extra, int32_t K,
                                     float* weights_sum, float* depth, float* image, float* extra_out, float* weights,
                                     int32_t* sample_ray, inr_stream_t s) {
  INR_REQUIRE(rays && weights_sum && depth && image && N >= 0 && M >= 0, "bad argument");
  INR_REQUIRE(!sample_ray || weights, "sample_ray needs weights");
  INR_REQUIRE(!extra || (extra_out && weights && K > 0 && K <= 64), "extra needs extra_out, weights and 0 < K <= 64");
  INR_REQUIRE(!extra_out || M == 0 || (extra && weights), "extra_out needs extra and weights");
  if (N == 0) return INR_OK;
  INR_REQUIRE(M == 0 || (sigmas && rgbs && deltas), "null sample arrays");
  INR_REQUIRE(((uintptr_t)deltas & 7) == 0, "deltas must be 8-byte aligned");
  hipStream_t st = as_stream(s);
  k_composite_train_fwd<<<blocks_for(N * 64, kRayBlock), kRayBlock, 0, st>>>(sigmas, rgbs, deltas, rays, N, M, T_thresh,
                                                                             weights_sum, depth, image, weights, sample_ray);
  if (extra_out && K > 0)
    k_composite_train_extra_fwd<<<blocks_for(N * 64, kRayBlock), kRayBlock, 0, st>>>(weights, extra, rays, N, M, K,
                                                                                     extra_out, CeArgs{});
  return check_launch("composite_rays_train_forward");
}

int inr_composite_rays_extra_forward(const float* weights, const float* extra, const int32_t* rays, int64_t N, int64_t M,
                                     int32_t K, float* extra_out, const int64_t* labels, int32_t n_classes,
                                     int64_t ignore_index, float* grad_pix, void* workspace, float* loss_out,
                                     inr_stream_t s) {
  INR_REQUIRE(rays && extra_out && N >= 0 && M >= 0 && K > 0 && K <= 64, "bad argument");
  INR_REQUIRE(!labels || (grad_pix && workspace && loss_out && n_classes > 0 && n_classes <= K),
              "labels need grad_pix, workspace, loss_out and 0 < n_classes <= K");
  INR_REQUIRE(((uintptr_t)workspace & 15) == 0, "workspace must be 16-byte aligned");
  if (N == 0) return INR_OK;
  INR_REQUIRE(M == 0 || (weights && extra), "null sample arrays");
  hipStream_t st = as_stream(s);
  CeArgs ce{};
  if (labels) ce = CeArgs{labels, n_classes, ignore_index, grad_pix, reinterpret_cast<float4*>(workspace)};
  k_composite_train_extra_fwd<<<blocks_for(N * 64, kRayBlock), kRayBlock, 0, st>>>(weights, extra, rays, N, M, K, extra_out, ce);
  if (labels) k_ce_finalize<<<1, 1024, 0, st>>>(reinterpret_cast<const float4*>(workspace), N, loss_out);
  return check_launch("composite_rays_extra_forward");
}

int inr_composite_rays_train_backward(const float* grad_weights_sum, const float* grad_image,
                                      const float* grad_extra_out, const float* sigmas, const float* rgbs,
                                      const float* extra, const float* deltas, const int32_t* rays,
                                      const float* weights_sum, const float* image, const float* weights, int64_t N,
                                      int64_t M, float T_thresh, int32_t K, float* grad_sigmas, float* grad_rgbs,
                                      float* grad_extra, const int32_t* total_dev, inr_stream_t s) {
  (void)extra;
  INR_REQUIRE(rays && N >= 0 && M >= 0, "bad argument");
  INR_REQUIRE((grad_sigmas != nullptr) == (grad_rgbs != nullptr), "grad_sigmas and grad_rgbs go together");
  INR_REQUIRE(!grad_sigmas || (grad_image && weights_sum && image && (M == 0 || (sigmas && rgbs && deltas))), "null pointer");
  INR_REQUIRE(!grad_extra_out || M == 0 || (grad_extra && weights && K > 0 && K <= 64),
              "grad_extra_out needs grad_extra, weights and 0 < K <= 64");
  if (N == 0 || M == 0) return INR_OK;
  hipStream_t st = as_stream(s);
  if (grad_sigmas)
    k_composite_train_bwd<<<blocks_for(N * 64, kRayBlock), kRayBlock, 0, st>>>(grad_weights_sum, grad_image, sigmas,
                                                                               rgbs, deltas, rays, weights_sum, image, N, M,
                                                                               T_thresh, grad_sigmas, grad_rgbs, total_dev);
  if (grad_extra_out)
    k_composite_train_extra_bwd<<<blocks_for(N * 64, kRayBlock), kRayBlock, 0, st>>>(grad_extra_out, weights, rays, N,
                                                                                     M, K, grad_extra);
  return check_launch("composite_rays_train_backward");
}

}
```

### instance_nerf_amd/nerf/renderer.py

```python
import math
import os

import torch
import torch.nn as nn

from .. import _lib, raymarching
from .._lib import check, ptr, stream_ptr


def sample_pdf(bins, weights, n_samples, det=False):
    weights = weights + 1e-5
    pdf = weights / torch.sum(weights, -1, keepdim=True)
    cdf = torch.cat([torch.zeros_like(pdf[..., :1]), torch.cumsum(pdf, -1)], -1)
    if det:
        u = torch.linspace(0.5 / n_samples, 1 - 0.5 / n_samples, steps=n_samples, device=weights.device)
        u = u.expand(list(cdf.shape[:-1]) + [n_samples])
    else:
        u = torch.rand(list(cdf.shape[:-1]) + [n_samples], device=weights.device)
    u = u.contiguous()
    inds = torch.searchsorted(cdf, u, right=True)
    below = torch.max(torch.zeros_like(inds - 1), inds - 1)
    above = torch.min((cdf.shape[-1] - 1) * torch.ones_like(inds), inds)
    cdf_g = torch.stack([torch.gather(cdf, 1, below), torch.gather(cdf, 1, above)], -1)
    bins_g = torch.stack([torch.gather(bins, 1, below), torch.gather(bins, 1, above)], -1)
    denom = cdf_g[..., 1] - cdf_g[..., 0]
    denom = torch.where(denom < 1e-5, torch.ones_like(denom), denom)
    t = (u - cdf_g[..., 0]) / denom
    return bins_g[..., 0] + t * (bins_g[..., 1] - bins_g[..., 0])


class NeRFRenderer(nn.Module):
    min_staged_batch = 1 << 20

    def __init__(self, bound=1, cuda_ray=False, density_scale=1, min_near=0.2, density_thresh=0.01,
                 bg_radius=-1, grid_size=128):
        super().__init__()
        self.bound = bound
        self.cascade = 1 + math.ceil(math.log2(bound))
        self.grid_size = grid_size
        self.density_scale = density_scale
        self.min_near = min_near
        self.density_thresh = density_thresh
        self.bg_radius = bg_radius
        if bg_radius > 0:
            raise NotImplementedError("background sphere model is outside the hot path (SURVEY.md section 2)")
        aabb = torch.tensor([-bound, -bound, -bound, bound, bound, bound], dtype=torch.float32)
        self.register_buffer("aabb_train", aabb)
        self.register_buffer("aabb_infer", aabb.clone())
        self.cuda_ray = cuda_ray
        if cuda_ray:
            self.register_buffer("density_grid", torch.zeros(self.cascade, grid_size ** 3))
            self.register_buffer("density_bitfield", torch.zeros(self.cascade * grid_size ** 3 // 8, dtype=torch.uint8))
            self.mean_density = 0
            self.iter_density = 0
            self.register_buffer("step_counter", torch.zeros(16, 2, dtype=torch.int32))
            self.mean_count = 0
            self.local_step = 0
            self.last_counter = None

    @property
    def mean_density(self):
        pending = self.__dict__.get("_mean_density_dev")
        if pending is not None:
            self.__dict__["_mean_density"] = float(pending[0].item())
            self.__dict__["_mean_density_dev"] = None
        return self.__dict__.get("_mean_density", 0)

    @mean_density.setter
    def mean_density(self, value):
        self.__dict__["_mean_density_dev"] = None
        self.__dict__["_mean_density"] = value

    def forward(self, x, d):
        raise NotImplementedError()

    def density(self, x):
        raise NotImplementedError()

    def color(self, x, d, mask=None, **kwargs):
        raise NotImplementedError()

    def density_sigma(self, x):
        return self.density(x)["sigma"]

    def instance(self, x):
        return None

    def reset_extra_state(self):
        if not self.cuda_ray:
            return
        self.density_grid.zero_()
        self.mean_density = 0
        self.iter_density = 0
        self.step_counter.zero_()
        self.mean_count = 0
        self.local_step = 0

    def run(self, rays_o, rays_d, num_steps=128, upsample_steps=128, bg_color=None, perturb=False, **kwargs):
        prefix = rays_o.shape[:-1]
        rays_o = rays_o.contiguous().view(-1, 3).float()
        rays_d = rays_d.contiguous().view(-1, 3).float()
        N, device = rays_o.shape[0], rays_o.device
        aabb = self.aabb_train if self.training else self.aabb_infer
        nears, fars = raymarching.near_far_from_aabb(rays_o, rays_d, aabb, self.min_near)
        hit = (fars > nears) & (fars < 3.0e38)
        nears = torch.where(hit, nears, torch.zeros_like(nears)).unsqueeze(-1)
        fars = torch.where(hit, fars, torch.ones_like(fars)).unsqueeze(-1)

        z_vals = torch.linspace(0.0, 1.0, num_steps, device=device).unsqueeze(0)
        z_vals = nears + (fars - nears) * z_vals
        sample_dist = (fars - nears) / num_steps
        if perturb:
            z_vals = z_vals + (torch.rand(z_vals.shape, device=device) - 0.5) * sample_dist

        def positions(z):
            x = rays_o.unsqueeze(-2) + rays_d.unsqueeze(-2) * z.unsqueeze(-1)
            return torch.min(torch.max(x, aabb[:3]), aabb[3:])

        def weights_of(z, sigma):
            deltas = torch.cat([z[..., 1:] - z[..., :-1], sample_dist * torch.ones_like(z[..., :1])], dim=-1)
            alphas = 1 - torch.exp(-deltas * self.density_scale * sigma)
            shifted = torch.cat([torch.ones_like(alphas[..., :1]), 1 - alphas + 1e-15], dim=-1)
            return alphas * torch.cumprod(shifted, dim=-1)[..., :-1], deltas

        xyzs = positions(z_vals)
        den = {k: v.view(N, num_steps, -1) for k, v in self.density(xyzs.reshape(-1, 3)).items()}
        if upsample_steps > 0:
            with torch.no_grad():
                weights, deltas = weights_of(z_vals, den["sigma"].squeeze(-1))
                z_mid = z_vals[..., :-1] + 0.5 * deltas[..., :-1]
                new_z = sample_pdf(z_mid, weights[:, 1:-1], upsample_steps, det=not self.training).detach()
                new_xyzs = positions(new_z)
            new_den = {k: v.view(N, upsample_steps, -1) for k, v in self.density(new_xyzs.reshape(-1, 3)).items()}
            z_vals, order = torch.sort(torch.cat([z_vals, new_z], dim=1), dim=1)
            xyzs = torch.gather(torch.cat([xyzs, new_xyzs], dim=1), 1, order.unsqueeze(-1).expand(-1, -1, 3))
            den = {k: torch.gather(torch.cat([den[k], new_den[k]], dim=1), 1,
                                   order.unsqueeze(-1).expand(-1, -1, den[k].shape[-1])) for k in den}
        weights, _ = weights_of(z_vals, den["sigma"].squeeze(-1))
        weights = weights * hit.unsqueeze(-1)
        T = z_vals.shape[1]
        dirs = rays_d.unsqueeze(-2).expand(-1, T, -1)
        mask = (weights > 1e-4).reshape(-1)
        rgbs = self.color(xyzs.reshape(-1, 3), dirs.reshape(-1, 3), mask=mask,
                          geo_feat=den["geo_feat"].reshape(-1, den["geo_feat"].shape[-1])).view(N, T, 3)
        weights_sum = weights.sum(dim=-1)
        depth = torch.sum(weights * ((z_vals - nears) / (fars - nears)).clamp(0, 1), dim=-1)
        image = torch.sum(weights.unsqueeze(-1) * rgbs, dim=-2)
        if bg_color is None:
            bg_color = 1
        image = image + (1 - weights_sum).unsqueeze(-1) * bg_color
        results = {"image": image.view(*prefix, 3), "depth": depth.view(*prefix), "weights_sum": weights_sum.view(*prefix)}
        if getattr(self, "num_instances", 0) > 0:
            logits = self.instance(xyzs.reshape(-1, 3)).view(N, T, -1)
            results["instance"] = torch.sum(weights.detach().unsqueeze(-1) * logits, dim=-2).view(*prefix, -1)
        return results

    def _instance_for_compositing(self, x):
        return self.instance(x)

    def run_cuda(self, rays_o, rays_d, dt_gamma=0, bg_color=None, perturb=False, force_all_rays=False,
                 max_steps=1024, T_thresh=1e-4, infer_mode="auto", noises=None, field_gate=None, ce_labels=None,
                 ce_ignore_index=-1, mse_target=None, marched=None, ce_prune=False, **kwargs):
        prefix = rays_o.shape[:-1]
        rays_o = rays_o.contiguous().view(-1, 3).float()
        rays_d = rays_d.contiguous().view(-1, 3).float()
        N = rays_o.shape[0]
        device = rays_o.device
        aabb = self.aabb_train if self.training else self.aabb_infer
        if marched is not None and not (self.training and marched["n_rays"] == N
                                        and marched.get("grid_state", self.iter_density) == self.iter_density):
            self.drop_ahead(marched)
            marched = None
        if marched is not None:
            marched["consume"]()
            nears, fars = marched["nears"], marched["fars"]
        elif self.training and ce_prune and ce_labels is not None:
            nears, fars = raymarching.near_far_from_aabb(rays_o, rays_d, aabb, self.min_near, skip_labels=ce_labels,
                                                         ignore_index=ce_ignore_index)
        else:
            nears, fars = raymarching.near_far_from_aabb(rays_o, rays_d, aabb, self.min_near)
        if bg_color is None:
            bg_color = 1
        results = {}
        skipped_frac = None
        with_instance = getattr(self, "num_instances", 0) > 0
        if not self.training and infer_mode == "auto":
            infer_mode = "fused_terminate" if self._recent_skippable() > self.terminate_above else "fused"

        fused_inst = with_instance and getattr(self, "_fusable_inst", False) and hasattr(self, "instance_render")
        if (not self.training and infer_mode == "fused_terminate" and getattr(self, "_fusable", False)
                and (fused_inst or not with_instance)):
            counter = torch.zeros(2, dtype=torch.int32, device=device)
            xyzs, _, deltas, rays = raymarching.march_rays_patch(
                rays_o, rays_d, self.bound, self.density_bitfield, self.cascade, self.grid_size, nears, fars,
                dt_gamma, max_steps, noises=noises if perturb else None, counter=counter, table=True)
            if field_gate is not None:
                field_gate.acquire()
            weights_sum, depth, image, wbuf, evaluated = self.nerf_render(xyzs, deltas, rays, rays_d, T_thresh,
                                                                          want_weights=with_instance, normalised=True)
            if field_gate is not None:
                field_gate.release()
            if with_instance:
                if field_gate is not None:
                    field_gate.acquire()
                results["instance"] = self.instance_render(xyzs, rays, wbuf, normalised=True).view(*prefix, -1)
                if field_gate is not None:
                    field_gate.release()
            results["num_samples"] = counter
            results["num_evaluated"] = evaluated
            skipped_frac = (evaluated, int(xyzs.shape[0]), True)
        elif not self.training and infer_mode in ("fused", "fused_terminate"):
            counter = torch.zeros(2, dtype=torch.int32, device=device)
            table = (fused_inst or not with_instance) and getattr(self, "_fusable", False) and hasattr(self, "forward_table")
            early = {}

            def while_waiting():
                early["skippable"] = torch.zeros(1, dtype=torch.int64, device=device)
                if table and hasattr(self, "sh_table"):
                    early["shq"] = self.sh_table(rays_d)
            xyzs, dirs, deltas, rays = raymarching.march_rays_patch(
                rays_o, rays_d, self.bound, self.density_bitfield, self.cascade, self.grid_size, nears, fars,
                dt_gamma, max_steps, noises=noises if perturb else None, counter=counter, table=table,
                while_waiting=while_waiting)
            if field_gate is not None:
                field_gate.acquire()
            sigmas, rgbs = self.forward_table(xyzs, dirs, rays_d, shq=early.get("shq")) if table else self(xyzs, dirs)
            if field_gate is not None:
                field_gate.release()
            if self.density_scale != 1:
                sigmas = self.density_scale * sigmas
            skippable = early["skippable"]
            if fused_inst:
                weights_sum, depth, image, wbuf = raymarching.composite_rays_patch(sigmas, rgbs, deltas, rays, T_thresh,
                                                                                  return_weights=True, skippable=skippable)
                if field_gate is not None:
                    field_gate.acquire()
                results["instance"] = self.instance_render(xyzs, rays, wbuf, normalised=table).view(*prefix, -1)
                if field_gate is not None:
                    field_gate.release()
            else:
                extra = self._instance_for_compositing(xyzs) if with_instance else None
                out = raymarching.composite_rays_patch(sigmas, rgbs, deltas, rays, T_thresh, extra=extra,
                                                       skippable=skippable)
                weights_sum, depth, image = out[0], out[1], out[2]
                if with_instance:
                    results["instance"] = out[3][:, :self.num_instances].reshape(*prefix, -1)
            results["num_samples"] = counter
            if table:
                results["frame_path"] = getattr(self, "last_frame_path", "fused")
            skipped_frac = (skippable, int(xyzs.shape[0]), False)
        elif self.training or infer_mode == "fused_raymajor":
            if marched is not None:
                counter = marched["counter"]
                xyzs, dirs, deltas, rays = marched["xyzs"], marched["dirs"], marched["deltas"], marched["rays"]
            else:
                if self.training:
                    counter = self.step_counter[self.local_step % 16]
                    self.local_step += 1
                    mean_count = self.mean_count
                else:
                    counter = torch.zeros(2, dtype=torch.int32, device=device)
                    mean_count = -1
                    force_all_rays = True
                xyzs, dirs, deltas, rays = raymarching.march_rays_train(
                    rays_o, rays_d, self.bound, self.density_bitfield, self.cascade, self.grid_size, nears, fars,
                    counter, mean_count, perturb, 128, force_all_rays, dt_gamma, max_steps, noises=noises)
            if self.training:
                self.last_counter = counter
            head = with_instance and getattr(self, "instance_head_available", lambda x: False)(xyzs)
            shaded = None
            if (marched is not None and marched.get("shaded") is not None and head and self.shade_ahead_applies()
                    and marched["T_thresh"] == float(T_thresh) and marched["density_scale"] == float(self.density_scale)):
                shaded = marched["shaded"]
            else:
                sigmas, rgbs = self(xyzs, dirs)
                if self.density_scale != 1:
                    sigmas = self.density_scale * sigmas
            if head:
                weights_sum, depth, image, wbuf, sample_ray = shaded if shaded is not None else raymarching.composite_rays_train(
                    sigmas, rgbs, deltas, rays, T_thresh, return_weights=True, total_dev=counter)
                if ce_labels is not None:
                    inst, results["instance_ce"] = self.instance_head_train(
                        xyzs, wbuf, sample_ray, rays, n_dev=counter, ce_labels=ce_labels.reshape(-1),
                        ce_ignore_index=ce_ignore_index)
                else:
                    inst = self.instance_head_train(xyzs, wbuf, sample_ray, rays, n_dev=counter)
                results["instance"] = inst[:, :self.num_instances].reshape(*prefix, -1)
            else:
                extra = self._instance_for_compositing(xyzs) if with_instance else None
                out = raymarching.composite_rays_train(sigmas, rgbs, deltas, rays, T_thresh, extra=extra,
                                                       total_dev=counter)
                weights_sum, depth, image = out[0], out[1], out[2]
                if with_instance:
                    results["instance"] = out[3][:, :self.num_instances].reshape(*prefix, -1)
            results["num_samples"] = counter
        elif infer_mode == "wavefront":
            dtype = torch.float32
            weights_sum = torch.zeros(N, dtype=dtype, device=device)
            depth = torch.zeros(N, dtype=dtype, device=device)
            image = torch.zeros(N, 3, dtype=dtype, device=device)
            K = getattr(self, "num_instances", 0)
            inst = torch.zeros(N, K, dtype=dtype, device=device) if with_instance else None
            n_alive = N
            rays_alive = torch.arange(n_alive, dtype=torch.int32, device=device)
            rays_t = nears.clone()
            step = 0
            evaluated = 0
            while step < max_steps and n_alive > 0:
                n_step = max(min(N // n_alive, 8), 1)
                xyzs, dirs, deltas = raymarching.march_rays(n_alive, n_step, rays_alive, rays_t, rays_o, rays_d,
                                                            self.bound, self.density_bitfield, self.cascade,
                                                            self.grid_size, nears, fars, 128, perturb, dt_gamma,
                                                            max_steps)
                sigmas, rgbs = self(xyzs, dirs)
                sigmas = self.density_scale * sigmas
                extra = self.instance(xyzs) if with_instance else None
                raymarching.composite_rays(n_alive, n_step, rays_alive, rays_t, sigmas, rgbs, deltas, weights_sum,
                                           depth, image, T_thresh, extra=extra, extra_acc=inst)
                evaluated += n_alive * n_step
                rays_alive, n_alive = raymarching.compact_alive(rays_alive, n_alive)
                step += n_step
            if with_instance:
                results["instance"] = inst.view(*prefix, -1)
        else:
            raise ValueError(f"unknown infer_mode {infer_mode!r}")

        if not self.training and skipped_frac is not None:
            self._note_skippable(*skipped_frac)
        t_start = None
        if not self.training and infer_mode in ("fused", "fused_terminate", "fused_raymajor"):
            t_start = nears
            if perturb and noises is not None:
                dt_min = 2 * math.sqrt(3) / max_steps
                dt_max = 2 * math.sqrt(3) * 2 ** (self.cascade - 1) / self.grid_size
                t_start = nears + torch.clamp(nears * dt_gamma, dt_min, dt_max) * noises.to(nears)
        bg3 = self._bg_triplet(bg_color)
        flows = torch.is_grad_enabled() and (image.requires_grad or weights_sum.requires_grad)
        bg_per_ray = torch.is_tensor(bg_color) and bg_color.is_cuda and bg_color.numel() == 3 * N
        if (self.training and mse_target is not None and flows and t_start is None and image.is_cuda
                and 0 < N <= raymarching.FINISH_MSE_MAX_RAYS and (bg3 is not None or bg_per_ray)):
            image, depth, results["image_mse"] = raymarching.finish_rays_mse(
                image, weights_sum, depth, nears, fars, bg3 if bg3 is not None else bg_color, mse_target)
        elif bg3 is not None and not (torch.is_grad_enabled() and (image.requires_grad or weights_sum.requires_grad)):
            lib = _lib.load()
            src_i, src_d = image.detach().contiguous(), depth.detach().contiguous()
            image = torch.empty_like(src_i) if self.training else src_i
            depth = torch.empty_like(src_d) if self.training else src_d
            check(lib.inr_finish_rays(ptr(src_i, torch.float32, "image"), ptr(src_d, torch.float32, "depth"),
                                      ptr(weights_sum.detach().contiguous(), torch.float32, "weights_sum"),
                                      ptr(nears, torch.float32, "nears"), ptr(fars, torch.float32, "fars"),
                                      ptr(t_start, torch.float32, "t0", allow_none=True),
                                      bg3[0], bg3[1], bg3[2], N, ptr(image), ptr(depth), stream_ptr()), "finish_rays")
        else:
            if isinstance(bg_color, (list, tuple)):
                bg_color = image.new_tensor(bg_color)
            image = image + (1 - weights_sum).unsqueeze(-1) * bg_color
            if t_start is not None:
                depth = depth + t_start * weights_sum.detach()
            depth = torch.clamp(depth - nears, min=0) / (fars - nears)
        results["image"] = image.view(*prefix, 3)
        results["depth"] = depth.view(*prefix)
        results["weights_sum"] = weights_sum.view(*prefix)
        return results

    terminate_above = 0.50

    def _note_skippable(self, counter, total, counts_evaluated):
        if not counter.is_cuda:
            v = float(counter.reshape(-1)[0]) / max(total, 1)
            self._skippable_value = 1.0 - v if counts_evaluated else v
            return
        d = self.__dict__
        if "_skippable_free" not in d:
            d["_skippable_free"] = [torch.empty(1, dtype=torch.int64, pin_memory=True) for _ in range(4)]
            d["_skippable_pending"] = []
        self._recent_skippable()
        if not d["_skippable_free"]:
            return
        host = d["_skippable_free"].pop()
        host.copy_(counter.reshape(-1)[:1].view(torch.int64), non_blocking=True)
        ev = torch.cuda.Event()
        ev.record()
        d["_skippable_pending"].append((ev, host, total, counts_evaluated))

    def _recent_skippable(self):
        d = self.__dict__
        pending = d.get("_skippable_pending", [])
        while pending and pending[0][0].query():
            _, host, total, counts_evaluated = pending.pop(0)
            v = float(int(host[0])) / max(total, 1)
            d["_skippable_value"] = 1.0 - v if counts_evaluated else v
            d["_skippable_free"].append(host)
        return d.get("_skippable_value", 0.0)

    @staticmethod
    def _bg_triplet(bg_color):
        if isinstance(bg_color, (int, float)):
            return (float(bg_color),) * 3
        if isinstance(bg_color, (list, tuple)) and len(bg_color) == 3 and all(isinstance(c, (int, float)) for c in bg_color):
            return tuple(float(c) for c in bg_color)
        return None

    @torch.no_grad()
    def mark_untrained_grid(self, poses, intrinsic, S=64):
        if not self.cuda_ray:
            return
        if not torch.is_tensor(poses):
            poses = torch.as_tensor(poses)
        dev = self.density_grid.device
        poses = poses.to(dev).float().contiguous().view(-1, 16)
        fx, fy, cx, cy = [float(v) for v in intrinsic]
        check(_lib.load().inr_mark_untrained_grid(ptr(poses, torch.float32, "poses", allow_none=poses.shape[0] == 0),
                                                  poses.shape[0], fx, fy, cx, cy, self.grid_size, self.cascade,
                                                  float(self.bound), ptr(self.density_grid, torch.float32, "density_grid"),
                                                  stream_ptr()), "mark_untrained_grid")

    def shade_ahead_applies(self):
        if not (getattr(self, "num_instances", 0) > 0 and getattr(self, "_fusable", False)
                and hasattr(self, "_nerf_params") and hasattr(self, "instance_head_train")):
            return False
        if any(p.requires_grad for p in self._nerf_params()):
            return False
        inst = [self.instance_encoder.embeddings] + [l.weight for l in self.instance_net]
        return bool(self._fusable_inst and self.fused_instance_train and self.fused_instance_head
                    and all(p.requires_grad for p in inst))

    @torch.no_grad()
    def march_ahead(self, rays_o, rays_d, dt_gamma=0, perturb=False, max_steps=1024, stream=None, shade=False,
                    T_thresh=1e-4, bufs=None, counter=None, skip_labels=None, ignore_index=-1):
        if not (self.cuda_ray and self.training and self.mean_count > 0 and rays_o.is_cuda):
            return None
        rays_o_in, rays_d_in = rays_o, rays_d
        rays_o = rays_o.contiguous().view(-1, 3).float()
        rays_d = rays_d.contiguous().view(-1, 3).float()
        N = rays_o.shape[0]
# ... 42 lines not shown
            if side is not main:
                done = torch.cuda.Event()
                done.record(side)
        out = {"n_rays": N, "key": (rays_o.data_ptr(), rays_d.data_ptr(), N), "rays_o": rays_o_in, "rays_d": rays_d_in,
               "nears": nears, "fars": fars, "xyzs": xyzs, "dirs": dirs, "deltas": deltas, "rays": rays, "counter": counter,
               "shaded": shaded, "T_thresh": float(T_thresh), "density_scale": float(self.density_scale),
               "slot_taken": slot_taken, "slot_index": slot_index, "grid_state": self.iter_density,
               "skip_labels": skip_labels}

        def consume():
            cur = torch.cuda.current_stream()
            if done is not None and side is not cur:
                cur.wait_event(done)
        out["consume"] = consume
        return out

    def drop_ahead(self, marched):
        if marched is not None and marched.get("slot_taken") and self.local_step > 0:
            if marched.get("slot_index", -1) == (self.local_step - 1) % 16:
                self.local_step -= 1
            marched["slot_taken"] = False

    @torch.no_grad()
    def update_extra_state(self, decay=0.95, S=128):
        if not self.cuda_ray:
            return
        lib = _lib.load()
        dev = self.density_bitfield.device
        H, C = self.grid_size, self.cascade
        n_cells = H ** 3
        st = stream_ptr()
        total_step = min(16, self.local_step)
        counted = None
        if total_step > 0:
            host = self.__dict__.get("_count_host")
            if host is None:
                host = self.__dict__["_count_host"] = torch.empty(1, dtype=torch.int64).pin_memory()
            host.copy_(self.step_counter[:total_step, 0].sum(0, keepdim=True, dtype=torch.int64), non_blocking=True)
            counted = torch.cuda.Event()
            counted.record()
        mean_sum = torch.zeros(1, dtype=torch.float64, device=dev)
        grid = self.density_grid
        full = self.iter_density < 16
        for cas in range(C):
            bnd = float(min(2 ** cas, self.bound))
            if full:
                idx, m = None, n_cells
            else:
                n = n_cells // 4
                u = torch.rand(4 * n, dtype=torch.float32, device=dev)
                idx = torch.empty(2 * n, dtype=torch.int32, device=dev)
                work = torch.empty(lib.inr_occ_sample_workspace_bytes(n_cells) // 8 + 1, dtype=torch.int64, device=dev)
                check(lib.inr_occ_sample_cells(ptr(grid[cas], torch.float32, "density_grid"), n_cells, ptr(u), n, ptr(idx),
                                               ptr(work), st), "occ_sample_cells")
                m = 2 * n
            xyz = torch.empty(m, 3, dtype=torch.float32, device=dev)
            noise = torch.rand_like(xyz)
            check(lib.inr_occ_cell_positions(ptr(idx, torch.int32, "morton_idx", allow_none=True),
                                             ptr(noise, torch.float32, "noise"), m, H, bnd, ptr(xyz), st),
                  "occ_cell_positions")
            sigma = self.density_sigma(xyz).reshape(-1).detach().float().contiguous()
            tmp = None if full else torch.empty(n_cells, dtype=torch.float32, device=dev)
            check(lib.inr_occ_update(ptr(grid[cas], torch.float32, "density_grid"), ptr(sigma, torch.float32, "sigma"),
                                     ptr(idx, torch.int32, "morton_idx", allow_none=True), n_cells, m, float(decay),
                                     float(self.density_scale), ptr(tmp, allow_none=True), ptr(mean_sum), st),
                  "occ_update")
        stats = torch.empty(2, dtype=torch.float64, device=dev)
        check(lib.inr_packbits_mean(ptr(grid, torch.float32, "density_grid"), C * n_cells, ptr(mean_sum),
                                    float(self.density_thresh), ptr(self.density_bitfield, torch.uint8, "density_bitfield"),
                                    None, ptr(self.step_counter, torch.int32, "step_counter"), max(total_step, 1),
                                    self.step_counter.stride(0), ptr(stats), st), "packbits_mean")
        self.iter_density += 1
        self.__dict__["_mean_density_dev"] = stats
        if counted is not None:
            counted.synchronize()
            self.mean_count = int(float(host[0]) / total_step)
        self.local_step = 0

    def render(self, rays_o, rays_d, staged=False, max_ray_batch=4096, **kwargs):
        _run = self.run_cuda if self.cuda_ray else self.run
        B, N = rays_o.shape[:2]
        if self.cuda_ray:
            max_ray_batch = max(int(max_ray_batch), int(self.min_staged_batch))
        if staged and N > max_ray_batch:
            if not self.training and kwargs.get("infer_mode", "auto") == "auto":
                kwargs = dict(kwargs, infer_mode="fused_terminate" if self._recent_skippable() > self.terminate_above else "fused")
            chunks = {}
            for b in range(B):
                head = 0
                while head < N:
                    tail = min(head + max_ray_batch, N)
                    r = _run(rays_o[b:b + 1, head:tail], rays_d[b:b + 1, head:tail], **kwargs)
                    for k, v in r.items():
                        if torch.is_tensor(v) and v.dim() >= 2 and v.shape[:2] == (1, tail - head):
                            chunks.setdefault((k, b), []).append(v)
                    head += max_ray_batch
            keys = sorted({k for k, _ in chunks})
            n_chunks = (N + max_ray_batch - 1) // max_ray_batch
            keys = [k for k in keys if all(len(chunks.get((k, b), ())) == n_chunks for b in range(B))]
            return {k: torch.cat([torch.cat(chunks[(k, b)], 1) for b in range(B)], 0) for k in keys}
        return _run(rays_o, rays_d, **kwargs)


class FramePipeline:

    def __init__(self, net, device=None):
        self.net = net
        self.streams = [torch.cuda.Stream(device=device), torch.cuda.Stream(device=device)]
        self._turn = 0
        self._field_done = None
        self.open()

    def open(self):
        raymarching.set_overlap_placement(os.environ.get("INR_PIPELINE_PLACEMENT", "1") != "0")

    def acquire(self):
        if self._field_done is not None:
            torch.cuda.current_stream().wait_event(self._field_done)

    def release(self):
        self._field_done = torch.cuda.Event()
        self._field_done.record(torch.cuda.current_stream())

    def next_stream(self):
        st = self.streams[self._turn]
        self._turn ^= 1
        return st

    def render(self, rays_o, rays_d, stream=None, **kwargs):
        if kwargs.pop("staged", False):
            raise RuntimeError("FramePipeline renders a whole view per call (staged=False)")
        if stream is None:
            stream = self.next_stream()
            stream.wait_stream(torch.cuda.current_stream())
            rays_o.record_stream(stream)
            rays_d.record_stream(stream)
        with torch.cuda.stream(stream):
            out = self.net.render(rays_o, rays_d, staged=False, field_gate=self, **kwargs)
        out["stream"] = stream
        return out

    def synchronize(self):
        for st in self.streams:
            st.synchronize()

    def close(self):
        self.synchronize()
        raymarching.set_overlap_placement(False)

    def __enter__(self):
        return self

    def __exit__(self, *exc):
        self.close()
        return False
```

### instance_nerf_amd/nerf/utils.py

```python
import math
import os
import time

import numpy as np
import torch
import torch.distributed as dist

from .. import _lib


_PATCH_INDS = {}


SUPER_TILE = int(os.environ.get("INR_SUPER_TILE", "0"))


def patch_order(H, W, patch, device, super_tile=None):
    st = SUPER_TILE if super_tile is None else super_tile
    key = (H, W, patch, st, str(device))
    if key not in _PATCH_INDS:
        jj, ii = torch.meshgrid(torch.arange(H), torch.arange(W), indexing="ij")
        ii, jj = ii.reshape(-1), jj.reshape(-1)
        npx = (W + patch - 1) // patch
        k = ((jj // patch) * npx + (ii // patch))
# ... 677 lines not shown
        self.ckpt_path = self.best_path = None
        if self.workspace is not None:
            self.ckpt_path = os.path.join(self.workspace, "checkpoints")
            self.best_path = os.path.join(self.ckpt_path, f"{self.name}.pth")
        if self.workspace is not None and use_checkpoint != "scratch":
            if use_checkpoint in ("latest", "latest_model"):
                self.load_checkpoint(model_only=use_checkpoint == "latest_model")
            elif use_checkpoint == "best":
                if self.best_path and os.path.exists(self.best_path):
                    self.load_checkpoint(self.best_path)
                else:
                    self.load_checkpoint()
            else:
                self.load_checkpoint(use_checkpoint)

    def log(self, *args, **kwargs):
        if self.local_rank == 0 and not self.mute:
            print(*args, **kwargs)

    def _lr_step(self):
        if self.lr_scheduler is not None:
            return
        f = 0.1 ** min(self.global_step / self.iters, 1)
        for g, b in zip(self.optimizer.param_groups, self.base_lrs):
            g["lr"] = b * f

    def _render_kwargs(self):
        return vars(self.opt) if self.opt is not None else {}

    def train_step(self, data):
        bg_color = self.bg_color
        gt = None
        if self.stage == "nerf":
            images = data["images"]
            gt = images
            if images.shape[-1] == 4:
                bg_color = torch.rand_like(images[..., :3])
                gt = images[..., :3] * images[..., 3:] + bg_color * (1 - images[..., 3:])
        extra = {}
        if self.stage == "instance" and getattr(self.model, "cuda_ray", False) and data["rays_o"].is_cuda:
            extra["ce_labels"] = data["masks"]
            extra["ce_prune"] = self.prune_ignored
        if (self.stage == "nerf" and self._default_criterion and getattr(self.model, "cuda_ray", False)
                and data["rays_o"].is_cuda):
            extra["mse_target"] = gt
        ahead = self._ahead
        if ahead is not None:
            self._ahead = None
            if (ahead["rays_o"] is data["rays_o"] and ahead["rays_d"] is data["rays_d"]
                    and ahead.get("skip_labels") is self._skip_labels(data)):
                extra["marched"] = ahead
            elif hasattr(self.model, "drop_ahead"):
                self.model.drop_ahead(ahead)
        outputs = self.model.render(data["rays_o"], data["rays_d"], staged=False, bg_color=bg_color, perturb=True,
                                    force_all_rays=False, **extra, **self._render_kwargs())
        if self.stage == "nerf":
            pred = outputs["image"]
            loss = outputs["image_mse"] if "image_mse" in outputs else self.criterion(pred, gt).mean()
            return pred, gt, loss
        logits = outputs["instance"]
        K = logits.shape[-1]
        if "instance_ce" in outputs:
            loss = outputs["instance_ce"]
        elif logits.is_cuda and K <= 64 and logits.dtype == torch.float32:
            from .. import raymarching
            loss = raymarching.cross_entropy(logits.reshape(-1, K), data["masks"].reshape(-1), ignore_index=-1)
        else:
            loss = torch.nn.functional.cross_entropy(logits.reshape(-1, K), data["masks"].reshape(-1).long(), ignore_index=-1)
        return logits, data["masks"], loss

    @staticmethod
    def _as_image(t, data, channels=None):
        if "H" in data and "W" in data and t.dim() >= 2 and t.shape[1] == int(data["H"]) * int(data["W"]):
            tail = t.shape[2:]
            return t.reshape(t.shape[0], int(data["H"]), int(data["W"]), *tail)
        return t

    def _render_view(self, data, **kwargs):
        rays_o, rays_d = data["rays_o"], data["rays_d"]
        H, W = int(data.get("H", 0) or 0), int(data.get("W", 0) or 0)
        if not (getattr(self.model, "cuda_ray", False) and rays_o.is_cuda and rays_o.dim() == 3 and H * W == rays_o.shape[1]
                and H % 4 == 0 and W % 4 == 0):
            return self.model.render(rays_o, rays_d, **kwargs)
        inds = patch_order(H, W, 4, rays_o.device)
        out = self.model.render(rays_o[:, inds].contiguous(), rays_d[:, inds].contiguous(), **kwargs)
        for k, v in list(out.items()):
            if torch.is_tensor(v) and v.dim() >= 2 and v.shape[1] == H * W:
                back = torch.empty_like(v)
                back[:, inds] = v
                out[k] = back
        return out

    @torch.no_grad()
    def eval_step(self, data):
        outputs = self._render_view(data, staged=True, bg_color=self.bg_color, perturb=False, **self._render_kwargs())
        return self._eval_outputs(data, outputs)

    def _eval_outputs(self, data, outputs):
        if self.stage == "nerf":
            images = data["images"]
            flat = images.reshape(images.shape[0], -1, images.shape[-1])
            gt = flat[..., :3] * flat[..., 3:] + self.bg_color * (1 - flat[..., 3:]) if flat.shape[-1] == 4 else flat
            loss = self.criterion(outputs["image"], gt).mean()
            return (self._as_image(outputs["image"], data), self._as_image(outputs["depth"], data),
                    self._as_image(gt, data), loss)
        logits = outputs["instance"]
        K = logits.shape[-1]
        masks = data["masks"].reshape(logits.shape[0], -1)
        loss = torch.nn.functional.cross_entropy(logits.reshape(-1, K), masks.reshape(-1).long(), ignore_index=-1)
        return (self._as_image(logits.argmax(-1), data), self._as_image(outputs["depth"], data),
                self._as_image(masks, data), loss)

    @torch.no_grad()
    def test_step(self, data, bg_color=None, perturb=False):
        outputs = self._render_view(data, staged=True, bg_color=self.bg_color if bg_color is None else bg_color,
                                    perturb=perturb, **self._render_kwargs())
        return self._test_outputs(data, outputs)

    def _test_outputs(self, data, outputs):
        inst = outputs.get("instance")
        return (self._as_image(outputs["image"], data), self._as_image(outputs["depth"], data),
                None if inst is None else self._as_image(inst, data))

    pipeline_views = True

    @torch.no_grad()
    def render_sequence(self, loader, pipeline=None, **kwargs):
        kw = dict(staged=True, bg_color=self.bg_color, perturb=False)
        kw.update(self._render_kwargs())
        kw.update(kwargs)
        use = self.pipeline_views if pipeline is None else bool(pipeline)
        use = use and getattr(self.model, "cuda_ray", False) and self.device.type == "cuda"
        if not use:
            for data in loader:
                yield data, self._render_view(data, **kw)
            return
        from .renderer import FramePipeline
        pipe = self.__dict__.get("_frame_pipe")
        if pipe is None or pipe.net is not self.model:
            pipe = self.__dict__["_frame_pipe"] = FramePipeline(self.model, self.device)
        pipe.open()
        try:
            pending = None
            for data in loader:
                cur = torch.cuda.current_stream()
                st = pipe.next_stream()
                st.wait_stream(cur)
                for k in ("rays_o", "rays_d"):
                    if torch.is_tensor(data.get(k)) and data[k].is_cuda:
                        data[k].record_stream(st)
                with torch.cuda.stream(st):
                    out = self._render_view(data, field_gate=pipe, **kw)
                    done = torch.cuda.Event()
                    done.record(st)
                if pending is not None:
                    yield self._finish_view(*pending)
                pending = (data, out, done)
            if pending is not None:
                yield self._finish_view(*pending)
        finally:
            pipe.close()

    @staticmethod
    def _finish_view(data, out, done):
        done.synchronize()
        cur = torch.cuda.current_stream()
        for v in out.values():
            if torch.is_tensor(v) and v.is_cuda:
                v.record_stream(cur)
        return data, out

    GRAPH_ALIGN = 16384

    def _graph_capacity(self, mean_count):
# ... 510 lines not shown
```

### instance_nerf_amd/raymarching.py

```python
import math

import torch

from . import _lib
from ._lib import check, ptr, stream_ptr

F32, I32, U8 = torch.float32, torch.int32, torch.uint8

SAMPLE_CAP = int(__import__("os").environ.get("INR_SAMPLE_CAP", "1024"))
SAMPLE_CAP_TRAIN = int(__import__("os").environ.get("INR_SAMPLE_CAP_TRAIN", "0"))


def _f(t):
    return t.contiguous().float() if (t.dtype != F32 or not t.is_contiguous()) else t


def set_overlap_placement(on):
    check(_lib.load().inr_set_overlap_placement(1 if on else 0), "set_overlap_placement")


def set_march_mode(mode):
    code = {None: -1, "auto": -1, "lane_per_ray": 0, "wave_per_ray": 1}[mode]
    check(_lib.load().inr_set_march_mode(code), "set_march_mode")

# ... 80 lines not shown
                  "weights": torch.empty(n_samples, dtype=F32, device=device),
                  "sample_ray": torch.empty(n_samples, dtype=I32, device=device)})
    return b


def march_rays_train(rays_o, rays_d, bound, density_bitfield, C, H, nears, fars, step_counter=None,
                     mean_count=-1, perturb=False, align=-1, force_all_rays=False, dt_gamma=0, max_steps=1024,
                     noises=None, separate_buffers=False, out=None):
    lib = _lib.load()
    rays_o, rays_d = _f(rays_o).view(-1, 3), _f(rays_d).view(-1, 3)
    dev = rays_o.device
    N = rays_o.shape[0]
    nears, fars = _f(nears), _f(fars)
    if noises is None:
        if not perturb:
            noises = None
        elif out is not None:
            noises = torch.rand(N, dtype=F32, device=dev, out=out["noises"])
        else:
            noises = torch.rand(N, dtype=F32, device=dev)
    else:
        noises = _f(noises)
    if step_counter is None:
        step_counter = torch.zeros(2, dtype=I32, device=dev)
    cap = SAMPLE_CAP_TRAIN
    if out is not None:
        if force_all_rays or mean_count <= 0 or out["n_rays"] != N or out["n_samples"] < int(mean_count):
            raise RuntimeError("march_rays_train(out=) needs the steady state and buffers of the batch's size")
        rays, ws = out["rays"], out["ws"]
    else:
        rays = torch.empty(N, 3, dtype=I32, device=dev)
        ws = torch.empty(lib.inr_march_workspace_bytes(N, cap) // 8 + 1, dtype=torch.int64, device=dev)
    args = (ptr(rays_o, F32, "rays_o"), ptr(rays_d, F32, "rays_d"), ptr(density_bitfield, U8, "density_bitfield"),
            float(bound), float(dt_gamma), int(max_steps), N, int(C), int(H))
    check(lib.inr_march_rays_train_count(*args, ptr(nears, F32, "nears"), ptr(fars, F32, "fars"),
                                         ptr(noises, F32, "noises", allow_none=True), ptr(rays),
                                         ptr(step_counter, I32, "step_counter"), ptr(ws), cap, stream_ptr()),
          "march_rays_train_count")
    if force_all_rays or mean_count <= 0:
        M = int(step_counter[0].item())
    else:
        M = int(mean_count)
    if align > 0:
        M += align - M % align if M % align else 0
    alloc = torch.empty if lib.inr_march_write_fills_unowned_rows(N, cap, int(max_steps)) else torch.zeros
    if out is not None:
        if alloc is not torch.empty or M > out["n_samples"]:
            raise RuntimeError("march_rays_train(out=) needs the staged marcher (it clears unowned rows itself)")
        buf = out["buf"]
        xyzs, dirs, deltas = buf[:M * 3].view(M, 3), buf[M * 3:M * 6].view(M, 3), buf[M * 6:M * 8].view(M, 2)
    elif separate_buffers:
        xyzs, dirs, deltas = (alloc(M, 3, dtype=F32, device=dev), alloc(M, 3, dtype=F32, device=dev),
                              alloc(M, 2, dtype=F32, device=dev))
    else:
        buf = alloc(M * 8, dtype=F32, device=dev)
        xyzs, dirs, deltas = buf[:M * 3].view(M, 3), buf[M * 3:M * 6].view(M, 3), buf[M * 6:].view(M, 2)
    check(lib.inr_march_rays_train_write(*args, M, ptr(nears), ptr(fars), ptr(noises, F32, "noises", allow_none=True),
                                         ptr(rays), ptr(xyzs), ptr(dirs), ptr(deltas), ptr(ws), cap, stream_ptr()),
          "march_rays_train_write")
    return xyzs, dirs, deltas, rays


GROUP = 16


_PINNED_COUNT = {}


def _read_count(counter, while_waiting=None):
    key = counter.device.index
    host = _PINNED_COUNT.get(key)
    if host is None:
        host = _PINNED_COUNT[key] = torch.empty(2, dtype=I32, pin_memory=True)
    host.copy_(counter[:2], non_blocking=True)
    ev = torch.cuda.Event()
    ev.record()
    if while_waiting is not None:
        while_waiting()
    ev.synchronize()
    return int(host[0])


def march_rays_patch(rays_o, rays_d, bound, density_bitfield, C, H, nears, fars, dt_gamma=0, max_steps=1024,
                     noises=None, counter=None, table=False, while_waiting=None):
    lib = _lib.load()
    rays_o, rays_d = _f(rays_o).view(-1, 3), _f(rays_d).view(-1, 3)
    dev = rays_o.device
    N = rays_o.shape[0]
    nears, fars = _f(nears), _f(fars)
    noises = _f(noises) if noises is not None else None
    if counter is None:
        counter = torch.zeros(2, dtype=I32, device=dev)
    rays = torch.empty(N, 3, dtype=I32, device=dev)
    cap = SAMPLE_CAP
    ws = torch.empty(lib.inr_march_workspace_bytes(N, cap) // 8 + 1, dtype=torch.int64, device=dev)
    args = (ptr(rays_o, F32, "rays_o"), ptr(rays_d, F32, "rays_d"), ptr(density_bitfield, U8, "density_bitfield"),
            float(bound), float(dt_gamma), int(max_steps), N, int(C), int(H))
    check(lib.inr_march_rays_train_count(*args, ptr(nears, F32, "nears"), ptr(fars, F32, "fars"),
                                         ptr(noises, F32, "noises", allow_none=True), ptr(rays),
                                         ptr(counter, I32, "counter"), ptr(ws), cap, stream_ptr()),
          "march_rays_train_count")
    M = _read_count(counter, while_waiting)
    xyzs = torch.empty(M, 3, dtype=F32, device=dev)
    dirs = None if table else torch.empty(M, 3, dtype=F32, device=dev)
    ray_ids = torch.empty(M, dtype=I32, device=dev) if table else None
    deltas = torch.empty(M, 2, dtype=F32, device=dev)
    check(lib.inr_march_rays_patch_write(*args, M, ptr(nears), ptr(fars), ptr(noises, F32, "noises", allow_none=True),
                                         ptr(rays), ptr(xyzs, allow_none=M == 0), ptr(dirs, allow_none=True),
                                         ptr(deltas, allow_none=M == 0), ptr(ws), cap,
                                         ptr(ray_ids, allow_none=True), 1 if table else 0, stream_ptr()),
          "march_rays_patch_write")
    return xyzs, (ray_ids if table else dirs), deltas, rays


def composite_rays_patch(sigmas, rgbs, deltas, rays, T_thresh=1e-4, extra=None, return_weights=False, skippable=None):
    lib = _lib.load()
    sigmas, rgbs, deltas = _f(sigmas), _f(rgbs), _f(deltas)
    dev = rays.device
    N, M = rays.shape[0], sigmas.shape[0]
    K = 0 if extra is None else extra.shape[1]
    ws = torch.empty(N, dtype=F32, device=dev)
    depth = torch.empty(N, dtype=F32, device=dev)
    image = torch.empty(N, 3, dtype=F32, device=dev)
    extra_out = torch.empty(N, K, dtype=F32, device=dev) if K else None
    wbuf = torch.empty(max(M, 1), dtype=F32, device=dev) if (K or return_weights) else None
    none_ok = M == 0
    check(lib.inr_composite_rays_patch_forward(
        ptr(sigmas, F32, "sigmas", allow_none=none_ok), ptr(rgbs, F32, "rgbs", allow_none=none_ok),
        ptr(deltas, F32, "deltas", allow_none=none_ok), ptr(rays, I32, "rays"), N, M, float(T_thresh),
        ptr(_f(extra) if extra is not None else None, allow_none=True), K, ptr(ws), ptr(depth), ptr(image),
        ptr(extra_out, allow_none=True), ptr(wbuf, allow_none=True), ptr(skippable, torch.int64, "skippable", allow_none=True),
        stream_ptr()), "composite_rays_patch_forward")
    out = (ws, depth, image) + ((extra_out,) if K else ())
    return out + ((wbuf,) if return_weights else ())


def patch_slots(rays):
    r = rays.cpu().long()
    N = r.shape[0]
    cnt, off = r[:, 2], r[:, 1]
    pad = (-N) % GROUP
    c = torch.cat([cnt, torch.zeros(pad, dtype=torch.long)]).view(-1, GROUP)
    base = torch.cat([off, torch.zeros(pad, dtype=torch.long)]).view(-1, GROUP)[:, 0]
    out = []
    for g in range(c.shape[0]):
        cg = c[g]
        kmax = int(cg.max())
        if kmax == 0:
            continue
        k = torch.arange(kmax)[:, None]
        act = cg[None, :] > k
        nact = act.sum(1)
        S = base[g] + torch.cat([torch.zeros(1, dtype=torch.long), nact.cumsum(0)[:-1]])
        rank = act.long().cumsum(1) - act.long()
        slot = S[:, None] + rank
        for i in range(GROUP):
            out.append(slot[: int(cg[i]), i])
    return torch.cat(out) if out else torch.zeros(0, dtype=torch.long)


class _CompositeRaysTrain(torch.autograd.Function):
    @staticmethod
    def forward(ctx, sigmas, rgbs, extra, deltas, rays, T_thresh, want_weights=False, total_dev=None):
        lib = _lib.load()
        sigmas, rgbs, deltas = _f(sigmas), _f(rgbs), _f(deltas)
        dev = sigmas.device
        N = rays.shape[0]
        K = 0 if extra is None else extra.shape[1]
        if extra is not None:
            extra = _f(extra)
        ws = torch.empty(N, dtype=F32, device=dev)
        depth = torch.empty(N, dtype=F32, device=dev)
        image = torch.empty(N, 3, dtype=F32, device=dev)
        extra_out = torch.empty(N, K, dtype=F32, device=dev) if K else None
        wbuf = torch.empty(sigmas.shape[0], dtype=F32, device=dev) if (K or want_weights) else None
        sample_ray = torch.empty(sigmas.shape[0], dtype=I32, device=dev) if want_weights else None
        check(lib.inr_composite_rays_train_forward(
            ptr(sigmas, F32, "sigmas"), ptr(rgbs, F32, "rgbs"), ptr(deltas, F32, "deltas"), ptr(rays, I32, "rays"),
            N, sigmas.shape[0], float(T_thresh), ptr(extra, F32, "extra", allow_none=True), K, ptr(ws), ptr(depth),
            ptr(image),
            ptr(extra_out, allow_none=True), ptr(wbuf, allow_none=True), ptr(sample_ray, allow_none=True), stream_ptr()),
            "composite_rays_train_forward")
        ctx.save_for_backward(sigmas, rgbs, extra, deltas, rays, ws, image, wbuf, total_dev)
        ctx.T_thresh = T_thresh
        ctx.K = K
        ctx.set_materialize_grads(False)
        if ctx.needs_input_grad[0] or ctx.needs_input_grad[1]:
            ctx.mark_non_differentiable(depth)
        else:
            ctx.mark_non_differentiable(depth, ws, image)
        out = (ws, depth, image) + ((extra_out,) if K else ())
        if want_weights:
            ctx.mark_non_differentiable(wbuf, sample_ray)
            out = out + (wbuf, sample_ray)
        ctx.n_out = len(out)
        return out

    @staticmethod
    def backward(ctx, g_ws, g_depth, g_image, *rest):
        g_extra = rest[0] if ctx.K else None
        lib = _lib.load()
        sigmas, rgbs, extra, deltas, rays, ws, image, wbuf, total_dev = ctx.saved_tensors
        N = rays.shape[0]
        K = ctx.K
        dev = sigmas.device
        need_field = ctx.needs_input_grad[0] or ctx.needs_input_grad[1]
        gs = gc = None
        if need_field:
            g_ws = _f(g_ws) if g_ws is not None else None
            g_image = _f(g_image) if g_image is not None else torch.zeros(N, 3, dtype=F32, device=dev)
            alloc = torch.empty_like if total_dev is not None else torch.zeros_like
            gs = alloc(sigmas)
            gc = alloc(rgbs)
        ge = None
        if K and g_extra is not None and ctx.needs_input_grad[2]:
# ... 177 lines not shown
```

Baseline: 6430 Msamples/s.

## Fuse patch-order permutation and near/far computation into march and composite kernels

Inference rendering used to gather rays into 4x4 patch order, render them, and scatter every output back with separate torch copies. It now passes the permutation index into the march count/write, composite and finish kernels, which read rays through the index and write results straight to their original pixel positions. The ray-box near/far calculation is also folded into the march count kernel. This removes the gather and scatter passes and one kernel launch, but the frame path skips the cooperative march kernel and the indexed reads may be less coalesced.

```diff
diff --git a/include/inr.h b/include/inr.h
--- a/include/inr.h
+++ b/include/inr.h
@@ -103,6 +103,27 @@
                                      float* extra_out , float* weights ,
                                      uint64_t* skippable ,
                                      inr_stream_t s);
+int inr_march_rays_frame_count(const float* rays_o, const float* rays_d, const int64_t* order, const float* aabb,
+                               float min_near, const uint8_t* bitfield, float bound, float dt_gamma,
+                               int32_t max_steps, int64_t N, int32_t cascade, int32_t H,
+                               const float* noises , float* nears , float* fars ,
+                               int32_t* rays, int32_t* counter, void* workspace, int32_t sample_cap, inr_stream_t s);
+int inr_march_rays_frame_write(const float* rays_o, const float* rays_d, const int64_t* order,
+                               const uint8_t* bitfield, float bound, float dt_gamma, int32_t max_steps, int64_t N,
+                               int32_t cascade, int32_t H, int64_t M, const float* nears, const float* fars,
+                               const float* noises , const int32_t* rays, float* xyzs,
+                               float* dirs , float* deltas, const void* workspace,
+                               int32_t sample_cap, int32_t* ray_ids , int32_t normalise,
+                               inr_stream_t s);
+int inr_composite_rays_frame_forward(const float* sigmas, const float* rgbs, const float* deltas,
+                                     const int32_t* rays, const int64_t* order, int64_t N, int64_t M, float T_thresh,
+                                     const float* extra , int32_t K, float* weights_sum,
+                                     float* depth, float* image, float* extra_out , float* weights ,
+                                     uint64_t* skippable , inr_stream_t s);
+int inr_finish_rays_frame(const float* image , const float* depth , const float* weights_sum,
+                          const float* nears, const float* fars, const float* t0 ,
+                          const int64_t* order, float bg_r, float bg_g, float bg_b, int64_t N, float* image_out,
+                          float* depth_out, inr_stream_t s);
 int inr_project_masks_patch(const float* xyzs, const float* weights, const int32_t* rays, int64_t N, int64_t M,
                             const uint32_t* mask_words, int32_t W, int32_t L, int32_t H, const float* bbox ,
                             int32_t k_total, int32_t k_base, int32_t k_count, float* out, inr_stream_t s);
diff --git a/instance_nerf_amd/_lib.py b/instance_nerf_amd/_lib.py
--- a/instance_nerf_amd/_lib.py
+++ b/instance_nerf_amd/_lib.py
@@ -75,6 +75,13 @@
     "inr_nerf_forward_table_sliced_workspace_bytes": (c_int64, [c_int64]),
     "inr_nerf_forward_table_sliced": (c_int32, [P, P, P, c_int64, c_float, P, POINTER(GridDesc), P, c_float, P, P, P, P]),
     "inr_composite_rays_patch_forward": (c_int32, [P, P, P, P, c_int64, c_int64, c_float, P, c_int32, P, P, P, P, P, P, P]),
+    "inr_march_rays_frame_count": (c_int32, [P, P, P, P, c_float, P, c_float, c_float, c_int32, c_int64, c_int32, c_int32,
+                                             P, P, P, P, P, P, c_int32, P]),
+    "inr_march_rays_frame_write": (c_int32, [P, P, P, P, c_float, c_float, c_int32, c_int64, c_int32, c_int32,
+                                             c_int64, P, P, P, P, P, P, P, P, c_int32, P, c_int32, P]),
+    "inr_composite_rays_frame_forward": (c_int32, [P, P, P, P, P, c_int64, c_int64, c_float, P, c_int32, P, P, P, P, P, P,
+                                                   P]),
+    "inr_finish_rays_frame": (c_int32, [P, P, P, P, P, P, P, c_float, c_float, c_float, c_int64, P, P, P]),
     "inr_project_masks_patch": (c_int32, [P, P, P, c_int64, c_int64, P, c_int32, c_int32, c_int32, P, c_int32, c_int32, c_int32,
                                           P, P]),
     "inr_march_rays": (c_int32, [c_int64, c_int32, P, P, P, P, c_float, c_float, c_int32, c_int32, c_int32,
diff --git a/instance_nerf_amd/csrc/raymarch.hip b/instance_nerf_amd/csrc/raymarch.hip
--- a/instance_nerf_amd/csrc/raymarch.hip
+++ b/instance_nerf_amd/csrc/raymarch.hip
@@ -15,16 +15,10 @@
 constexpr int kRayBlock = 256;
 constexpr float kSqrt3x2 = 3.4641016151377544f;
 
-__global__ void __launch_bounds__(kRayBlock) k_near_far(const float* __restrict__ rays_o,
-                                                        const float* __restrict__ rays_d,
-                                                        const float* __restrict__ aabb, int64_t N,
-                                                        float min_near, float* __restrict__ nears,
-                                                        float* __restrict__ fars,
-                                                        const int64_t* __restrict__ labels, int64_t ignore) {
-  const int64_t n = (int64_t)blockIdx.x * blockDim.x + threadIdx.x;
-  if (n >= N) return;
+__device__ __forceinline__ void ray_box(const float* __restrict__ rays_o, const float* __restrict__ rays_d, int64_t n,
+                                        const float* __restrict__ aabb, float min_near, bool miss, float& near_out,
+                                        float& far_out) {
   float near = -INFINITY, far = INFINITY;
-  bool miss = labels != nullptr && labels[n] == ignore;
 #pragma unroll
   for (int a = 0; a < 3; ++a) {
     const float o = rays_o[n * 3 + a];
@@ -38,8 +32,23 @@
     far = hi < far ? hi : far;
   }
   if (near < min_near) near = min_near;
-  nears[n] = miss ? 3.402823466e+38f : near;
-  fars[n] = miss ? 3.402823466e+38f : far;
+  near_out = miss ? 3.402823466e+38f : near;
+  far_out = miss ? 3.402823466e+38f : far;
+}
+
+__global__ void __launch_bounds__(kRayBlock) k_near_far(const float* __restrict__ rays_o,
+                                                        const float* __restrict__ rays_d,
+                                                        const float* __restrict__ aabb, int64_t N,
+                                                        float min_near, float* __restrict__ nears,
+                                                        float* __restrict__ fars,
+                                                        const int64_t* __restrict__ labels, int64_t ignore) {
+  const int64_t n = (int64_t)blockIdx.x * blockDim.x + threadIdx.x;
+  if (n >= N) return;
+  const bool miss = labels != nullptr && labels[n] == ignore;
+  float near, far;
+  ray_box(rays_o, rays_d, n, aabb, min_near, miss, near, far);
+  nears[n] = near;
+  fars[n] = far;
 }
 
 __global__ void __launch_bounds__(kRayBlock) k_get_rays(const float* __restrict__ poses, int64_t B, float fx, float fy,
@@ -325,6 +334,13 @@
   return near + step_dt(P, near) * noise;
 }
 
+struct FrameRays {
+  const int64_t* order;
+  const float* aabb;
+  float min_near;
+  float *nears, *fars;
+};
+
 __global__ void __launch_bounds__(kRayBlock) k_march_count(MarchParams P, const float* __restrict__ rays_o,
                                                            const float* __restrict__ rays_d, int64_t N,
                                                            int max_steps, const float* __restrict__ nears,
@@ -332,7 +348,8 @@
                                                            const float* __restrict__ noises,
                                                            int32_t* __restrict__ counts,
                                                            int32_t* __restrict__ block_sums,
-                                                           uint32_t* __restrict__ mask, int cap_words) {
+                                                           uint32_t* __restrict__ mask, int cap_words,
+                                                           FrameRays F) {
   __shared__ int32_t wsum[kRayBlock / 64];
   __shared__ uint32_t lut[1024];
   for (int i = threadIdx.x; i < P.H; i += kRayBlock) lut[i] = expand_bits10((uint32_t)i);
@@ -341,13 +358,23 @@
   const int64_t n = (int64_t)blockIdx.x * blockDim.x + threadIdx.x;
   int cnt = 0;
   if (n < N) {
-    const Ray r = load_ray(rays_o, rays_d, n);
-    const float t0 = start_t(P, nears[n], noises ? noises[n] : 0.0f);
+    const int64_t src = F.order ? F.order[n] : n;
+    const Ray r = load_ray(rays_o, rays_d, src);
+    float near, far;
+    if (F.aabb) {
+      ray_box(rays_o, rays_d, src, F.aabb, F.min_near, false, near, far);
+      F.nears[n] = near;
+      F.fars[n] = far;
+    } else {
+      near = nears[n];
+      far = fars[n];
+    }
+    const float t0 = start_t(P, near, noises ? noises[n] : 0.0f);
     if (cap_words > 0) {
       uint32_t word = 0;
       int widx = 0, cand = 0;
       bool ok = true;
-      cnt = march_ray_any(P, r, t0, fars[n], max_steps,
+      cnt = march_ray_any(P, r, t0, far, max_steps,
                       [&](float, float, float, float, float, float) {
                         const int w = cand >> 5;
                         if (w < cap_words) {
@@ -365,7 +392,7 @@
       if (widx < cap_words) mask[(int64_t)widx * N + n] = word;
       mask[(int64_t)cap_words * N + n] = ok ? 1u : 0u;
     } else {
-      cnt = march_ray_any(P, r, t0, fars[n], max_steps, [](float, float, float, float, float, float) {}, [] {}, morton);
+      cnt = march_ray_any(P, r, t0, far, max_steps, [](float, float, float, float, float, float) {}, [] {}, morton);
     }
     counts[n] = cnt;
   }
@@ -890,17 +917,19 @@
                                                      const float* __restrict__ weights_sum,
                                                      const float* __restrict__ nears, const float* __restrict__ fars,
                                                      const float* __restrict__ t0, float bg_r, float bg_g, float bg_b,
-                                                     int64_t N, float* image_out, float* depth_out) {
+                                                     int64_t N, float* image_out, float* depth_out,
+                                                     const int64_t* __restrict__ order) {
   const int64_t n = (int64_t)blockIdx.x * blockDim.x + threadIdx.x;
   if (n >= N) return;
-  const float ws = weights_sum[n];
+  const int64_t o = order ? order[n] : n;
+  const float ws = weights_sum[o];
   const float a = 1.0f - ws;
-  image_out[n * 3 + 0] = image[n * 3 + 0] + a * bg_r;
-  image_out[n * 3 + 1] = image[n * 3 + 1] + a * bg_g;
-  image_out[n * 3 + 2] = image[n * 3 + 2] + a * bg_b;
-  float d = depth[n];
+  image_out[o * 3 + 0] = image[o * 3 + 0] + a * bg_r;
+  image_out[o * 3 + 1] = image[o * 3 + 1] + a * bg_g;
+  image_out[o * 3 + 2] = image[o * 3 + 2] + a * bg_b;
+  float d = depth[o];
   if (t0) d = d + t0[n] * ws;
-  depth_out[n] = fmaxf(d - nears[n], 0.0f) / (fars[n] - nears[n]);
+  depth_out[o] = fmaxf(d - nears[n], 0.0f) / (fars[n] - nears[n]);
 }
 
 constexpr int kFinishMseThreads = 1024;
@@ -1341,14 +1370,16 @@
                                                                  float* __restrict__ xyzs, float* __restrict__ dirs,
                                                                  float* __restrict__ deltas,
                                                                  const uint32_t* __restrict__ mask, int cap_words,
-                                                                 int32_t* __restrict__ ray_ids, int normalise) {
+                                                                 int32_t* __restrict__ ray_ids, int normalise,
+                                                                 const int64_t* __restrict__ order) {
   const int64_t n = (int64_t)blockIdx.x * blockDim.x + threadIdx.x;
   const int off = n < N ? rays[n * 3 + 1] : 0;
   const int cnt = n < N ? rays[n * 3 + 2] : 0;
   GroupCursor cur;
   cur.init(cnt, off);
   if (cnt == 0 || (int64_t)cur.S + cur.total() > M) return;
-  const Ray r = load_ray(rays_o, rays_d, n);
+  const int64_t src = order ? order[n] : n;
+  const Ray r = load_ray(rays_o, rays_d, src);
   const float rb = 2.0f * P.bound;
   auto emit = [&](float px, float py, float pz, float dt, float delta, float) {
     const int64_t i = cur.next();
@@ -1357,8 +1388,8 @@
     }
     xyzs[i * 3 + 0] = px; xyzs[i * 3 + 1] = py; xyzs[i * 3 + 2] = pz;
     if (dirs) { dirs[i * 3 + 0] = r.dx; dirs[i * 3 + 1] = r.dy; dirs[i * 3 + 2] = r.dz; }
-    if (ray_ids) ray_ids[i] = (int32_t)n;
-    deltas[i * 2 + 0] = dt; deltas[i * 2 + 1] = delta;
+    if (ray_ids) ray_ids[i] = (int32_t)src;
+    reinterpret_cast<float2*>(deltas)[i] = make_float2(dt, delta);
   };
   const float t0 = start_t(P, nears[n], noises ? noises[n] : 0.0f);
   if (cap_words > 0 && mask[(int64_t)cap_words * N + n]) {
@@ -1375,7 +1406,8 @@
                                                                    float T_thresh, float* __restrict__ wbuf,
                                                                    float* __restrict__ weights_sum,
                                                                    float* __restrict__ depth, float* __restrict__ image,
-                                                                   unsigned long long* __restrict__ skippable) {
+                                                                   unsigned long long* __restrict__ skippable,
+                                                                   const int64_t* __restrict__ order) {
   const int64_t n = (int64_t)blockIdx.x * blockDim.x + threadIdx.x;
   const int lane = threadIdx.x & 63, g0 = lane & ~(kGroup - 1), rr = lane & (kGroup - 1);
   const int32_t rid = n < N ? rays[n * 3] : 0;
@@ -1432,8 +1464,9 @@
     }
   }
   if (n < N) {
-    weights_sum[rid] = ws; depth[rid] = dsum;
-    image[rid * 3] = r; image[rid * 3 + 1] = g; image[rid * 3 + 2] = b;
+    const int64_t row = order ? order[rid] : rid;
+    weights_sum[row] = ws; depth[row] = dsum;
+    image[row * 3] = r; image[row * 3 + 1] = g; image[row * 3 + 2] = b;
   }
   if (skippable) {
 #pragma unroll
@@ -1445,7 +1478,8 @@
 __global__ void __launch_bounds__(kRayBlock) k_composite_patch_extra(const float* __restrict__ wbuf,
                                                                      const float* __restrict__ extra,
                                                                      const int32_t* __restrict__ rays, int64_t N,
-                                                                     int64_t M, int K, float* __restrict__ extra_out) {
+                                                                     int64_t M, int K, float* __restrict__ extra_out,
+                                                                     const int64_t* __restrict__ order) {
   const int64_t n = ((int64_t)blockIdx.x * blockDim.x + threadIdx.x) >> 6;
   const int lane = threadIdx.x & 63;
   if (n >= N) return;
@@ -1475,7 +1509,7 @@
     const float w = wbuf[slot];
     if (lane < K && w != 0.0f) acc += w * extra[slot * K + lane];
   }
-  if (lane < K) extra_out[(int64_t)rid * K + lane] = acc;
+  if (lane < K) extra_out[(order ? order[rid] : (int64_t)rid) * K + lane] = acc;
 }
 
 struct MaskVolume {
@@ -1771,10 +1805,10 @@
 
 static size_t march_lds_pad() { return (size_t)inr::g_march_lds_pad; }
 
-int inr_march_rays_train_count(const float* rays_o, const float* rays_d, const uint8_t* bitfield, float bound,
-                               float dt_gamma, int32_t max_steps, int64_t N, int32_t cascade, int32_t H,
-                               const float* nears, const float* fars, const float* noises, int32_t* rays,
-                               int32_t* counter, void* workspace, int32_t sample_cap, inr_stream_t s) {
+static int march_count(const float* rays_o, const float* rays_d, const uint8_t* bitfield, float bound, float dt_gamma,
+                       int32_t max_steps, int64_t N, int32_t cascade, int32_t H, const float* nears, const float* fars,
+                       const float* noises, int32_t* rays, int32_t* counter, void* workspace, int32_t sample_cap,
+                       const FrameRays& F, inr_stream_t s) {
   INR_REQUIRE(rays_o && rays_d && bitfield && nears && fars && rays && counter && workspace, "null pointer");
   INR_REQUIRE(N > 0 && N < (1ll << 31), "N out of range");
   INR_REQUIRE(max_steps > 0 && cascade >= 1 && H >= 8 && H <= 1024, "bad grid parameters");
@@ -1785,7 +1819,7 @@
   int32_t* block_sums = counts + N;
   uint32_t* mask = reinterpret_cast<uint32_t*>(counts + ws_ints(N));
   hipStream_t st = as_stream(s);
-  if (use_coop(N, sample_cap)) {
+  if (!F.order && !F.aabb && use_coop(N, sample_cap)) {
     float* stage = use_stage(N, sample_cap, max_steps)
                        ? reinterpret_cast<float*>(reinterpret_cast<char*>(workspace) + stage_offset_bytes(N, sample_cap)) : nullptr;
     k_march_count_coop<<<blocks_for(N, kCoopRaysPerBlock), kCoopRaysPerBlock * 64, 0, st>>>(P, rays_o, rays_d, N, max_steps,
@@ -1794,11 +1828,30 @@
     k_scan_counts<<<1, 1024, 0, st>>>(counts, N, rays, counter);
     return check_launch("march_rays_train_count");
   }
-  k_march_count<<<nb, kRayBlock, march_lds_pad(), st>>>(P, rays_o, rays_d, N, max_steps, nears, fars, noises, counts, block_sums,
-                                          mask, cap_words_of(sample_cap));
+  k_march_count<<<nb, kRayBlock, march_lds_pad(), st>>>(P, rays_o, rays_d, N, max_steps, F.aabb ? nullptr : nears,
+                                                        F.aabb ? nullptr : fars, noises, counts, block_sums, mask,
+                                                        cap_words_of(sample_cap), F);
   k_scan_block_sums<<<1, 1024, 0, st>>>(block_sums, (int)nb, N, counter);
   k_finalize_offsets<<<nb, kRayBlock, 0, st>>>(counts, block_sums, N, rays);
   return check_launch("march_rays_train_count");
+}
+
+int inr_march_rays_train_count(const float* rays_o, const float* rays_d, const uint8_t* bitfield, float bound,
+                               float dt_gamma, int32_t max_steps, int64_t N, int32_t cascade, int32_t H,
+                               const float* nears, const float* fars, const float* noises, int32_t* rays,
+                               int32_t* counter, void* workspace, int32_t sample_cap, inr_stream_t s) {
+  return march_count(rays_o, rays_d, bitfield, bound, dt_gamma, max_steps, N, cascade, H, nears, fars, noises, rays, counter,
+                     workspace, sample_cap, FrameRays{nullptr, nullptr, 0.0f, nullptr, nullptr}, s);
+}
+
+int inr_march_rays_frame_count(const float* rays_o, const float* rays_d, const int64_t* order, const float* aabb,
+                               float min_near, const uint8_t* bitfield, float bound, float dt_gamma, int32_t max_steps,
+                               int64_t N, int32_t cascade, int32_t H, const float* noises, float* nears, float* fars,
+                               int32_t* rays, int32_t* counter, void* workspace, int32_t sample_cap, inr_stream_t s) {
+  INR_REQUIRE(order && aabb, "null pointer");
+  INR_REQUIRE(sample_cap > 0, "the frame marcher runs the lane-per-ray count pass (sample_cap > 0)");
+  return march_count(rays_o, rays_d, bitfield, bound, dt_gamma, max_steps, N, cascade, H, nears, fars, noises, rays, counter,
+                     workspace, sample_cap, FrameRays{order, aabb, min_near, nears, fars}, s);
 }
 
 int inr_march_rays_train_write(const float* rays_o, const float* rays_d, const uint8_t* bitfield, float bound,
@@ -1830,28 +1883,49 @@
   return check_launch("march_rays_train_write");
 }
 
+static int march_patch_write(const float* rays_o, const float* rays_d, const int64_t* order, const uint8_t* bitfield,
+                             float bound, float dt_gamma, int32_t max_steps, int64_t N, int32_t cascade, int32_t H, int64_t M,
+                             const float* nears, const float* fars, const float* noises, const int32_t* rays, float* xyzs,
+                             float* dirs, float* deltas, const void* workspace, int32_t sample_cap, int32_t* ray_ids,
+                             int32_t normalise, inr_stream_t s) {
+  INR_REQUIRE(rays_o && rays_d && bitfield && nears && fars && rays, "null pointer");
+  INR_REQUIRE(N > 0 && M >= 0, "bad sizes");
+  if (M == 0) return INR_OK;
+  INR_REQUIRE(M == 0 || (xyzs && deltas && (dirs || ray_ids)), "null output");
+  INR_REQUIRE(((uintptr_t)deltas & 7) == 0, "deltas must be 8-byte aligned");
+  const MarchParams P = make_params(bitfield, bound, dt_gamma, max_steps, cascade, H);
+  INR_REQUIRE(sample_cap == 0 || workspace, "sample_cap > 0 needs the workspace of the count pass");
+  const uint32_t* mask = sample_cap > 0 ? reinterpret_cast<const uint32_t*>(reinterpret_cast<const int32_t*>(workspace) + ws_ints(N)) : nullptr;
+  k_march_write_patch<<<blocks_for(N, kRayBlock), kRayBlock, march_lds_pad(), as_stream(s)>>>(P, rays_o, rays_d, N, M, nears, fars,
+                                                                                noises, rays, xyzs, dirs, deltas, mask,
+                                                                                cap_words_of(sample_cap), ray_ids, normalise,
+                                                                                order);
+  return check_launch("march_rays_patch_write");
+}
+
 int inr_march_rays_patch_write(const float* rays_o, const float* rays_d, const uint8_t* bitfield, float bound,
                                float dt_gamma, int32_t max_steps, int64_t N, int32_t cascade, int32_t H, int64_t M,
                                const float* nears, const float* fars, const float* noises, const int32_t* rays,
                                float* xyzs, float* dirs, float* deltas, const void* workspace, int32_t sample_cap,
                                int32_t* ray_ids, int32_t normalise, inr_stream_t s) {
-  INR_REQUIRE(rays_o && rays_d && bitfield && nears && fars && rays, "null pointer");
-  INR_REQUIRE(N > 0 && M >= 0, "bad sizes");
-  if (M == 0) return INR_OK;
-  INR_REQUIRE(M == 0 || (xyzs && deltas && (dirs || ray_ids)), "null output");
-  const MarchParams P = make_params(bitfield, bound, dt_gamma, max_steps, cascade, H);
-  INR_REQUIRE(sample_cap == 0 || workspace, "sample_cap > 0 needs the workspace of the count pass");
-  const uint32_t* mask = sample_cap > 0 ? reinterpret_cast<const uint32_t*>(reinterpret_cast<const int32_t*>(workspace) + ws_ints(N)) : nullptr;
-  k_march_write_patch<<<blocks_for(N, kRayBlock), kRayBlock, march_lds_pad(), as_stream(s)>>>(P, rays_o, rays_d, N, M, nears, fars,
-                                                                                noises, rays, xyzs, dirs, deltas, mask,
-                                                                                cap_words_of(sample_cap), ray_ids, normalise);
-  return check_launch("march_rays_patch_write");
-}
-
-int inr_composite_rays_patch_forward(const float* sigmas, const float* rgbs, const float* deltas, const int32_t* rays,
-                                     int64_t N, int64_t M, float T_thresh, const float* extra, int32_t K,
-                                     float* weights_sum, float* depth, float* image, float* extra_out,
-                                     float* weights, uint64_t* skippable, inr_stream_t s) {
+  return march_patch_write(rays_o, rays_d, nullptr, bitfield, bound, dt_gamma, max_steps, N, cascade, H, M, nears, fars,
+                           noises, rays, xyzs, dirs, deltas, workspace, sample_cap, ray_ids, normalise, s);
+}
+
+int inr_march_rays_frame_write(const float* rays_o, const float* rays_d, const int64_t* order, const uint8_t* bitfield,
+                               float bound, float dt_gamma, int32_t max_steps, int64_t N, int32_t cascade, int32_t H,
+                               int64_t M, const float* nears, const float* fars, const float* noises, const int32_t* rays,
+                               float* xyzs, float* dirs, float* deltas, const void* workspace, int32_t sample_cap,
+                               int32_t* ray_ids, int32_t normalise, inr_stream_t s) {
+  INR_REQUIRE(order, "null pointer");
+  return march_patch_write(rays_o, rays_d, order, bitfield, bound, dt_gamma, max_steps, N, cascade, H, M, nears, fars,
+                           noises, rays, xyzs, dirs, deltas, workspace, sample_cap, ray_ids, normalise, s);
+}
+
+static int composite_patch(const float* sigmas, const float* rgbs, const float* deltas, const int32_t* rays,
+                           const int64_t* order, int64_t N, int64_t M, float T_thresh, const float* extra, int32_t K,
+                           float* weights_sum, float* depth, float* image, float* extra_out, float* weights,
+                           uint64_t* skippable, inr_stream_t s) {
   INR_REQUIRE(N >= 0 && M >= 0, "bad sizes");
   if (N == 0) return INR_OK;
   INR_REQUIRE(rays && weights_sum && depth && image, "null pointer");
@@ -1861,11 +1935,29 @@
   hipStream_t st = as_stream(s);
   k_composite_patch_fwd<<<blocks_for(N, kRayBlock), kRayBlock, 0, st>>>(sigmas, rgbs, deltas, rays, N, M, T_thresh,
                                                                         weights, weights_sum, depth, image,
-                                                                        reinterpret_cast<unsigned long long*>(skippable));
+                                                                        reinterpret_cast<unsigned long long*>(skippable),
+                                                                        order);
   if (extra_out && K > 0)
     k_composite_patch_extra<<<blocks_for(N * 64, kRayBlock), kRayBlock, 0, st>>>(weights, extra, rays, N, M, K,
-                                                                                 extra_out);
+                                                                                 extra_out, order);
   return check_launch("composite_rays_patch_forward");
+}
+
+int inr_composite_rays_patch_forward(const float* sigmas, const float* rgbs, const float* deltas, const int32_t* rays,
+                                     int64_t N, int64_t M, float T_thresh, const float* extra, int32_t K,
+                                     float* weights_sum, float* depth, float* image, float* extra_out,
+                                     float* weights, uint64_t* skippable, inr_stream_t s) {
+  return composite_patch(sigmas, rgbs, deltas, rays, nullptr, N, M, T_thresh, extra, K, weights_sum, depth, image,
+                         extra_out, weights, skippable, s);
+}
+
+int inr_composite_rays_frame_forward(const float* sigmas, const float* rgbs, const float* deltas, const int32_t* rays,
+                                     const int64_t* order, int64_t N, int64_t M, float T_thresh, const float* extra,
+                                     int32_t K, float* weights_sum, float* depth, float* image, float* extra_out,
+                                     float* weights, uint64_t* skippable, inr_stream_t s) {
+  INR_REQUIRE(order, "null pointer");
+  return composite_patch(sigmas, rgbs, deltas, rays, order, N, M, T_thresh, extra, K, weights_sum, depth, image,
+                         extra_out, weights, skippable, s);
 }
 
 int inr_project_masks_patch(const float* xyzs, const float* weights, const int32_t* rays, int64_t N, int64_t M,
@@ -1949,8 +2041,19 @@
   if (N == 0) return INR_OK;
   INR_REQUIRE(image && depth && weights_sum && nears && fars && image_out && depth_out, "null pointer");
   k_finish_rays<<<blocks_for(N, 256), 256, 0, as_stream(s)>>>(image, depth, weights_sum, nears, fars, t0, bg_r, bg_g, bg_b,
-                                                              N, image_out, depth_out);
+                                                              N, image_out, depth_out, nullptr);
   return check_launch("finish_rays");
+}
+
+int inr_finish_rays_frame(const float* image, const float* depth, const float* weights_sum, const float* nears,
+                          const float* fars, const float* t0, const int64_t* order, float bg_r, float bg_g, float bg_b,
+                          int64_t N, float* image_out, float* depth_out, inr_stream_t s) {
+  INR_REQUIRE(N >= 0, "negative N");
+  if (N == 0) return INR_OK;
+  INR_REQUIRE(image && depth && weights_sum && nears && fars && order && image_out && depth_out, "null pointer");
+  k_finish_rays<<<blocks_for(N, 256), 256, 0, as_stream(s)>>>(image, depth, weights_sum, nears, fars, t0, bg_r, bg_g, bg_b,
+                                                              N, image_out, depth_out, order);
+  return check_launch("finish_rays_frame");
 }
 
 int inr_finish_rays_mse(const float* image, const float* depth, const float* weights_sum, const float* nears,
diff --git a/instance_nerf_amd/nerf/renderer.py b/instance_nerf_amd/nerf/renderer.py
--- a/instance_nerf_amd/nerf/renderer.py
+++ b/instance_nerf_amd/nerf/renderer.py
@@ -27,6 +27,17 @@
     denom = torch.where(denom < 1e-5, torch.ones_like(denom), denom)
     t = (u - cdf_g[..., 0]) / denom
     return bins_g[..., 0] + t * (bins_g[..., 1] - bins_g[..., 0])
+
+
+def render_permuted(run, rays_o, rays_d, order, **kwargs):
+    out = run(rays_o[:, order].contiguous(), rays_d[:, order].contiguous(), **kwargs)
+    n = order.numel()
+    for k, v in list(out.items()):
+        if torch.is_tensor(v) and v.dim() >= 2 and v.shape[1] == n:
+            back = torch.empty_like(v)
+            back[:, order] = v
+            out[k] = back
+    return out
 
 
 class NeRFRenderer(nn.Module):
@@ -160,7 +171,23 @@
 
     def run_cuda(self, rays_o, rays_d, dt_gamma=0, bg_color=None, perturb=False, force_all_rays=False,
                  max_steps=1024, T_thresh=1e-4, infer_mode="auto", noises=None, field_gate=None, ce_labels=None,
-                 ce_ignore_index=-1, mse_target=None, marched=None, ce_prune=False, **kwargs):
+                 ce_ignore_index=-1, mse_target=None, marched=None, ce_prune=False, order=None, **kwargs):
+        with_instance = getattr(self, "num_instances", 0) > 0
+        if not self.training and infer_mode == "auto":
+            infer_mode = "fused_terminate" if self._recent_skippable() > self.terminate_above else "fused"
+        fused_inst = with_instance and getattr(self, "_fusable_inst", False) and hasattr(self, "instance_render")
+        terminate = (not self.training and infer_mode == "fused_terminate" and getattr(self, "_fusable", False)
+                     and (fused_inst or not with_instance))
+        if order is not None:
+            native = (not self.training and not terminate and infer_mode in ("fused", "fused_terminate")
+                      and rays_o.is_cuda and rays_o.dim() == 3 and rays_o.shape[0] == 1 and raymarching.SAMPLE_CAP > 0
+                      and self._bg_triplet(1 if bg_color is None else bg_color) is not None)
+            if not native:
+                kw = dict(kwargs, dt_gamma=dt_gamma, bg_color=bg_color, perturb=perturb, force_all_rays=force_all_rays,
+                          max_steps=max_steps, T_thresh=T_thresh, infer_mode=infer_mode, noises=noises,
+                          field_gate=field_gate, ce_labels=ce_labels, ce_ignore_index=ce_ignore_index,
+                          mse_target=mse_target, marched=marched, ce_prune=ce_prune)
+                return render_permuted(self.run_cuda, rays_o, rays_d, order, **kw)
         prefix = rays_o.shape[:-1]
         rays_o = rays_o.contiguous().view(-1, 3).float()
         rays_d = rays_d.contiguous().view(-1, 3).float()
@@ -177,19 +204,16 @@
         elif self.training and ce_prune and ce_labels is not None:
             nears, fars = raymarching.near_far_from_aabb(rays_o, rays_d, aabb, self.min_near, skip_labels=ce_labels,
                                                          ignore_index=ce_ignore_index)
+        elif order is not None:
+            nears = fars = None
         else:
             nears, fars = raymarching.near_far_from_aabb(rays_o, rays_d, aabb, self.min_near)
         if bg_color is None:
             bg_color = 1
         results = {}
         skipped_frac = None
-        with_instance = getattr(self, "num_instances", 0) > 0
-        if not self.training and infer_mode == "auto":
-            infer_mode = "fused_terminate" if self._recent_skippable() > self.terminate_above else "fused"
-
-        fused_inst = with_instance and getattr(self, "_fusable_inst", False) and hasattr(self, "instance_render")
-        if (not self.training and infer_mode == "fused_terminate" and getattr(self, "_fusable", False)
-                and (fused_inst or not with_instance)):
+
+        if terminate:
             counter = torch.zeros(2, dtype=torch.int32, device=device)
             xyzs, _, deltas, rays = raymarching.march_rays_patch(
                 rays_o, rays_d, self.bound, self.density_bitfield, self.cascade, self.grid_size, nears, fars,
@@ -218,10 +242,13 @@
                 early["skippable"] = torch.zeros(1, dtype=torch.int64, device=device)
                 if table and hasattr(self, "sh_table"):
                     early["shq"] = self.sh_table(rays_d)
-            xyzs, dirs, deltas, rays = raymarching.march_rays_patch(
+            marched_frame = raymarching.march_rays_patch(
                 rays_o, rays_d, self.bound, self.density_bitfield, self.cascade, self.grid_size, nears, fars,
                 dt_gamma, max_steps, noises=noises if perturb else None, counter=counter, table=table,
-                while_waiting=while_waiting)
+                while_waiting=while_waiting, order=order, aabb=aabb, min_near=self.min_near)
+            xyzs, dirs, deltas, rays = marched_frame[:4]
+            if order is not None:
+                nears, fars = marched_frame[4:]
             if field_gate is not None:
                 field_gate.acquire()
             sigmas, rgbs = self.forward_table(xyzs, dirs, rays_d, shq=early.get("shq")) if table else self(xyzs, dirs)
@@ -232,16 +259,22 @@
             skippable = early["skippable"]
             if fused_inst:
                 weights_sum, depth, image, wbuf = raymarching.composite_rays_patch(sigmas, rgbs, deltas, rays, T_thresh,
-                                                                                  return_weights=True, skippable=skippable)
+                                                                                  return_weights=True, skippable=skippable,
+                                                                                  order=order)
                 if field_gate is not None:
                     field_gate.acquire()
-                results["instance"] = self.instance_render(xyzs, rays, wbuf, normalised=table).view(*prefix, -1)
+                inst = self.instance_render(xyzs, rays, wbuf, normalised=table)
                 if field_gate is not None:
                     field_gate.release()
+                if order is not None:
+                    back = torch.empty_like(inst)
+                    back[order] = inst
+                    inst = back
+                results["instance"] = inst.view(*prefix, -1)
             else:
                 extra = self._instance_for_compositing(xyzs) if with_instance else None
                 out = raymarching.composite_rays_patch(sigmas, rgbs, deltas, rays, T_thresh, extra=extra,
-                                                       skippable=skippable)
+                                                       skippable=skippable, order=order)
                 weights_sum, depth, image = out[0], out[1], out[2]
                 if with_instance:
                     results["instance"] = out[3][:, :self.num_instances].reshape(*prefix, -1)
@@ -346,11 +379,15 @@
             src_i, src_d = image.detach().contiguous(), depth.detach().contiguous()
             image = torch.empty_like(src_i) if self.training else src_i
             depth = torch.empty_like(src_d) if self.training else src_d
-            check(lib.inr_finish_rays(ptr(src_i, torch.float32, "image"), ptr(src_d, torch.float32, "depth"),
-                                      ptr(weights_sum.detach().contiguous(), torch.float32, "weights_sum"),
-                                      ptr(nears, torch.float32, "nears"), ptr(fars, torch.float32, "fars"),
-                                      ptr(t_start, torch.float32, "t0", allow_none=True),
-                                      bg3[0], bg3[1], bg3[2], N, ptr(image), ptr(depth), stream_ptr()), "finish_rays")
+            head = (ptr(src_i, torch.float32, "image"), ptr(src_d, torch.float32, "depth"),
+                    ptr(weights_sum.detach().contiguous(), torch.float32, "weights_sum"),
+                    ptr(nears, torch.float32, "nears"), ptr(fars, torch.float32, "fars"),
+                    ptr(t_start, torch.float32, "t0", allow_none=True))
+            tail = (bg3[0], bg3[1], bg3[2], N, ptr(image), ptr(depth), stream_ptr())
+            if order is not None:
+                check(lib.inr_finish_rays_frame(*head, ptr(order, torch.int64, "order"), *tail), "finish_rays_frame")
+            else:
+                check(lib.inr_finish_rays(*head, *tail), "finish_rays")
         else:
             if isinstance(bg_color, (list, tuple)):
                 bg_color = image.new_tensor(bg_color)
@@ -559,6 +596,13 @@
         B, N = rays_o.shape[:2]
         if self.cuda_ray:
             max_ray_batch = max(int(max_ray_batch), int(self.min_staged_batch))
+        order = kwargs.get("order")
+        if order is not None and (not self.cuda_ray or B != 1 or (staged and N > max_ray_batch)):
+            kwargs = {k: v for k, v in kwargs.items() if k != "order"}
+            return render_permuted(lambda o, d, **kw: self.render(o, d, staged, max_ray_batch, **kw), rays_o, rays_d,
+                                   order, **kwargs)
+        if order is None:
+            kwargs.pop("order", None)
         if staged and N > max_ray_batch:
             if not self.training and kwargs.get("infer_mode", "auto") == "auto":
                 kwargs = dict(kwargs, infer_mode="fused_terminate" if self._recent_skippable() > self.terminate_above else "fused")
diff --git a/instance_nerf_amd/nerf/utils.py b/instance_nerf_amd/nerf/utils.py
--- a/instance_nerf_amd/nerf/utils.py
+++ b/instance_nerf_amd/nerf/utils.py
@@ -783,14 +783,7 @@
         if not (getattr(self.model, "cuda_ray", False) and rays_o.is_cuda and rays_o.dim() == 3 and H * W == rays_o.shape[1]
                 and H % 4 == 0 and W % 4 == 0):
             return self.model.render(rays_o, rays_d, **kwargs)
-        inds = patch_order(H, W, 4, rays_o.device)
-        out = self.model.render(rays_o[:, inds].contiguous(), rays_d[:, inds].contiguous(), **kwargs)
-        for k, v in list(out.items()):
-            if torch.is_tensor(v) and v.dim() >= 2 and v.shape[1] == H * W:
-                back = torch.empty_like(v)
-                back[:, inds] = v
-                out[k] = back
-        return out
+        return self.model.render(rays_o, rays_d, order=patch_order(H, W, 4, rays_o.device), **kwargs)
 
     @torch.no_grad()
     def eval_step(self, data):
diff --git a/instance_nerf_amd/raymarching.py b/instance_nerf_amd/raymarching.py
--- a/instance_nerf_amd/raymarching.py
+++ b/instance_nerf_amd/raymarching.py
@@ -186,12 +186,20 @@
 
 
 def march_rays_patch(rays_o, rays_d, bound, density_bitfield, C, H, nears, fars, dt_gamma=0, max_steps=1024,
-                     noises=None, counter=None, table=False, while_waiting=None):
+                     noises=None, counter=None, table=False, while_waiting=None, order=None, aabb=None, min_near=0.2):
     lib = _lib.load()
     rays_o, rays_d = _f(rays_o).view(-1, 3), _f(rays_d).view(-1, 3)
     dev = rays_o.device
     N = rays_o.shape[0]
-    nears, fars = _f(nears), _f(fars)
+    frame = order is not None
+    if frame:
+        if order.dtype != torch.int64 or order.numel() != N or not order.is_contiguous() or order.device != dev:
+            raise RuntimeError("march_rays_patch: order must be a contiguous int64 permutation of the rays, on their device")
+        aabb = _f(aabb)
+        nears = torch.empty(N, dtype=F32, device=dev)
+        fars = torch.empty(N, dtype=F32, device=dev)
+    else:
+        nears, fars = _f(nears), _f(fars)
     noises = _f(noises) if noises is not None else None
     if counter is None:
         counter = torch.zeros(2, dtype=I32, device=dev)
@@ -200,24 +208,33 @@
     ws = torch.empty(lib.inr_march_workspace_bytes(N, cap) // 8 + 1, dtype=torch.int64, device=dev)
     args = (ptr(rays_o, F32, "rays_o"), ptr(rays_d, F32, "rays_d"), ptr(density_bitfield, U8, "density_bitfield"),
             float(bound), float(dt_gamma), int(max_steps), N, int(C), int(H))
-    check(lib.inr_march_rays_train_count(*args, ptr(nears, F32, "nears"), ptr(fars, F32, "fars"),
-                                         ptr(noises, F32, "noises", allow_none=True), ptr(rays),
-                                         ptr(counter, I32, "counter"), ptr(ws), cap, stream_ptr()),
-          "march_rays_train_count")
+    if frame:
+        check(lib.inr_march_rays_frame_count(args[0], args[1], ptr(order, torch.int64, "order"), ptr(aabb, F32, "aabb"),
+                                             float(min_near), *args[2:], ptr(noises, F32, "noises", allow_none=True),
+                                             ptr(nears), ptr(fars), ptr(rays), ptr(counter, I32, "counter"), ptr(ws),
+                                             cap, stream_ptr()), "march_rays_frame_count")
+    else:
+        check(lib.inr_march_rays_train_count(*args, ptr(nears, F32, "nears"), ptr(fars, F32, "fars"),
+                                             ptr(noises, F32, "noises", allow_none=True), ptr(rays),
+                                             ptr(counter, I32, "counter"), ptr(ws), cap, stream_ptr()),
+              "march_rays_train_count")
     M = _read_count(counter, while_waiting)
     xyzs = torch.empty(M, 3, dtype=F32, device=dev)
     dirs = None if table else torch.empty(M, 3, dtype=F32, device=dev)
     ray_ids = torch.empty(M, dtype=I32, device=dev) if table else None
     deltas = torch.empty(M, 2, dtype=F32, device=dev)
-    check(lib.inr_march_rays_patch_write(*args, M, ptr(nears), ptr(fars), ptr(noises, F32, "noises", allow_none=True),
-                                         ptr(rays), ptr(xyzs, allow_none=M == 0), ptr(dirs, allow_none=True),
-                                         ptr(deltas, allow_none=M == 0), ptr(ws), cap,
-                                         ptr(ray_ids, allow_none=True), 1 if table else 0, stream_ptr()),
-          "march_rays_patch_write")
+    tail = (M, ptr(nears), ptr(fars), ptr(noises, F32, "noises", allow_none=True), ptr(rays),
+            ptr(xyzs, allow_none=M == 0), ptr(dirs, allow_none=True), ptr(deltas, allow_none=M == 0), ptr(ws), cap,
+            ptr(ray_ids, allow_none=True), 1 if table else 0, stream_ptr())
+    if frame:
+        check(lib.inr_march_rays_frame_write(args[0], args[1], ptr(order), *args[2:], *tail), "march_rays_frame_write")
+        return xyzs, (ray_ids if table else dirs), deltas, rays, nears, fars
+    check(lib.inr_march_rays_patch_write(*args, *tail), "march_rays_patch_write")
     return xyzs, (ray_ids if table else dirs), deltas, rays
 
 
-def composite_rays_patch(sigmas, rgbs, deltas, rays, T_thresh=1e-4, extra=None, return_weights=False, skippable=None):
+def composite_rays_patch(sigmas, rgbs, deltas, rays, T_thresh=1e-4, extra=None, return_weights=False, skippable=None,
+                         order=None):
     lib = _lib.load()
     sigmas, rgbs, deltas = _f(sigmas), _f(rgbs), _f(deltas)
     dev = rays.device
@@ -229,12 +246,18 @@
     extra_out = torch.empty(N, K, dtype=F32, device=dev) if K else None
     wbuf = torch.empty(max(M, 1), dtype=F32, device=dev) if (K or return_weights) else None
     none_ok = M == 0
-    check(lib.inr_composite_rays_patch_forward(
-        ptr(sigmas, F32, "sigmas", allow_none=none_ok), ptr(rgbs, F32, "rgbs", allow_none=none_ok),
-        ptr(deltas, F32, "deltas", allow_none=none_ok), ptr(rays, I32, "rays"), N, M, float(T_thresh),
-        ptr(_f(extra) if extra is not None else None, allow_none=True), K, ptr(ws), ptr(depth), ptr(image),
-        ptr(extra_out, allow_none=True), ptr(wbuf, allow_none=True), ptr(skippable, torch.int64, "skippable", allow_none=True),
-        stream_ptr()), "composite_rays_patch_forward")
+    head = (ptr(sigmas, F32, "sigmas", allow_none=none_ok), ptr(rgbs, F32, "rgbs", allow_none=none_ok),
+            ptr(deltas, F32, "deltas", allow_none=none_ok), ptr(rays, I32, "rays"))
+    tail = (N, M, float(T_thresh), ptr(_f(extra) if extra is not None else None, allow_none=True), K, ptr(ws), ptr(depth),
+            ptr(image), ptr(extra_out, allow_none=True), ptr(wbuf, allow_none=True),
+            ptr(skippable, torch.int64, "skippable", allow_none=True), stream_ptr())
+    if order is not None:
+        if order.dtype != torch.int64 or order.numel() != N or not order.is_contiguous():
+            raise RuntimeError("composite_rays_patch: order must be a contiguous int64 permutation of the rays")
+        check(lib.inr_composite_rays_frame_forward(*head, ptr(order, torch.int64, "order"), *tail),
+              "composite_rays_frame_forward")
+    else:
+        check(lib.inr_composite_rays_patch_forward(*head, *tail), "composite_rays_patch_forward")
     out = (ws, depth, image) + ((extra_out,) if K else ())
     return out + ((wbuf,) if return_weights else ())
 
```

Result: no change. 6435 Msamples/s, median of 6 (+0.1%).
